# jcorsetti/oryon

Measured on AMD Instinct MI355X. Metric: image-pairs/sec end-to-end (feat+match+reg) @224², C=256; ADD(-S) parity, higher is better.
Workload: dtype f32

## Files before the change

include/oryon_hip.h:

```cpp
#ifndef ORYON_HIP_H
#define ORYON_HIP_H

#include <stddef.h>
#include <stdint.h>

#ifdef __cplusplus
extern "C" {
#endif

#define ORYON_OK 0
#define ORYON_ERR_INVALID_ARG (-1)
#define ORYON_ERR_HIP (-2)
#define ORYON_ERR_WORKSPACE (-3)
#define ORYON_ERR_NO_DEVICE (-4)
#define ORYON_ERR_STATE (-5)

#define ORYON_PAIR_OK 0
#define ORYON_PAIR_NO_MASK 1
#define ORYON_PAIR_NO_CORR 2

#define ORYON_MATCH_TILE 128

const char *oryon_version(void);
const char *oryon_last_error(void);
// ... 141 lines not shown
                     const float *cam_a, const float *cam_q, const int32_t *status, float *pcd_a, float *pcd_q,
                     int32_t *n_out, void *stream);

int oryon_lift_points(const float *depth, int H, int W, const float *cam9, const int32_t *x_idx, const int32_t *y_idx,
                      int n, float *out, void *stream);

int oryon_kabsch_batched(const float *A, const float *B, const float *w, int nb, int m, float *T, void *stream);

typedef struct oryon_pointdsc oryon_pointdsc_t;

typedef struct {
    int in_dim;
    int num_layers;
    int num_channels;
    int num_iterations;
    float ratio;
    float inlier_threshold;
    float sigma_d;
    int k;
    float nms_radius;
} oryon_pointdsc_config_t;

int oryon_pointdsc_create(oryon_pointdsc_t **handle, const oryon_pointdsc_config_t *cfg);
void oryon_pointdsc_destroy(oryon_pointdsc_t *handle);
int oryon_pointdsc_load_param(oryon_pointdsc_t *handle, const char *name, const float *data_host, int64_t numel);
int oryon_pointdsc_finalize(oryon_pointdsc_t *handle, void *stream);
size_t oryon_pointdsc_workspace_bytes(const oryon_pointdsc_t *handle, int B, int n_cap);
int oryon_pointdsc_register(oryon_pointdsc_t *handle, const float *src, const float *tgt, const int32_t *n, int B,
                            int n_cap, const int32_t *status_in, void *workspace, size_t workspace_bytes, float *T,
                            uint8_t *labels, int32_t *status_out, void *stream);
int oryon_pointdsc_encode(oryon_pointdsc_t *handle, const float *src, const float *tgt, const int32_t *n, int B,
                          int n_cap, void *workspace, size_t workspace_bytes, float *feat, float *confidence,
                          void *stream);
int oryon_pointdsc_seeds(oryon_pointdsc_t *handle, const float *src, const float *confidence, const int32_t *n, int B,
                         int n_cap, int S_cap, int32_t *seeds, int32_t *n_seeds, void *stream);
int oryon_pointdsc_hypotheses(oryon_pointdsc_t *handle, const float *src, const float *tgt, const float *feat,
                              const int32_t *n, const int32_t *seeds, const int32_t *n_seeds, int B, int n_cap,
                              int S_cap, void *workspace, size_t workspace_bytes, float *seed_T, float *fitness,
                              int32_t *best, void *stream);
int oryon_pointdsc_refine(oryon_pointdsc_t *handle, const float *src, const float *tgt, const int32_t *n, int B,
                          int n_cap, const float *T_in, float *T_out, uint8_t *labels, void *stream);

size_t oryon_ransac_workspace_bytes(int B, int n_cap, int max_iter);
int oryon_ransac_register(const float *src, const float *tgt, const int32_t *n, int B, int n_cap, int max_iter, double match_err,
                          double fix_percent, const int32_t *sample_idx, uint64_t seed, const int64_t *pair_key,
                          const int32_t *status_in, void *workspace, size_t workspace_bytes, float *T, int32_t *winner,
                          int32_t *exited, int32_t *counts, int32_t *status_out, void *stream);

size_t oryon_feature_loss_workspace_bytes(int B, int n_corr, int n_pool);
int oryon_feature_loss(const float *feat_a, const float *feat_q, int B, int C, int FH, int FW, const int32_t *corrs, int n_corr,
                       const int32_t *valid, const int32_t *pool, int n_pool, int pool_mode, float pos_margin, float neg_margin,
                       float neg_kernel, void *workspace, size_t workspace_bytes, float *d_pos, float *d_neg, int32_t *neg_idx,
                       float *pair_terms, float *losses, void *stream);
int oryon_mask_dice_sums(const float *logits, const int32_t *gt, int B, int H, int W, float threshold, double *sums, int32_t *mask,
                         int32_t *counts, void *stream);

size_t oryon_feature_loss_grad_workspace_bytes(int B, int C, int n_corr);
int oryon_feature_loss_grad(const float *feat_a, const float *feat_q, int B, int C, int FH, int FW, const int32_t *corrs, int n_corr,
                            const int32_t *valid, const int32_t *neg_idx, const float *d_pos, const float *d_neg, const float *g,
                            float pos_margin, float neg_margin, void *workspace, size_t workspace_bytes, float *grad_a, float *grad_q,
                            void *stream);
int oryon_mask_dice_grad(const float *logits, const int32_t *gt, int B, int H, int W, const double *sums, const float *g_mask,
                         float *grad_logits, void *stream);

typedef struct oryon_engine oryon_engine_t;
typedef struct {
    int B, C, FH, FW;
    int HA, WA, HQ, WQ;
    int layout;
    float dist_th;
    int n_corrs;
    int src_sampling;
    uint64_t seed;
    int round_f16;
    int n_slots;
    int overlap;
    int gather_sets;
    int reg_streams;
    int reg_lag;
    int screen;
    int sample_first;
    int x3_prefetch;
    int stream_roles;
    int solver;
    int ransac_max_iter;
    float ransac_match_err;
    float ransac_fix_percent;
} oryon_engine_config_t;
size_t oryon_engine_config_bytes(void);
size_t oryon_engine_arena_bytes(const oryon_engine_config_t *cfg, const oryon_pointdsc_t *solver);
int oryon_engine_create(oryon_engine_t **handle, const oryon_engine_config_t *cfg, oryon_pointdsc_t *solver, void *arena,
                        size_t arena_bytes);
void oryon_engine_destroy(oryon_engine_t *handle);
int oryon_engine_warm_streams(void);
int oryon_engine_set_stream_roles(oryon_engine_t *handle, int roles);
int oryon_engine_stream_roles(const oryon_engine_t *handle, int *roles);
int oryon_engine_buffer(const oryon_engine_t *handle, int slot, const char *name, size_t *offset, size_t *bytes);
int oryon_engine_geometry(const oryon_engine_t *handle, int *cap_a, int *cap_q, int *c_pad, int *n_cap);
int oryon_engine_submit(oryon_engine_t *handle, const float *feat_a, const float *feat_q, const int32_t *mask_a, const int32_t *mask_q,
                        const float *depth_a, const float *depth_q, const float *cam_a, const float *cam_q, const int64_t *pair_key,
                        int force_eager, int inputs_resident, void *caller_stream);
int oryon_engine_wait(oryon_engine_t *handle, int slot, void *caller_stream);
int oryon_engine_set_timing(oryon_engine_t *handle, int enable);
int oryon_engine_timing(oryon_engine_t *handle, int64_t step, float *out8);
int oryon_engine_elapsed(oryon_engine_t *handle, int64_t step_a, int event_a, int64_t step_b, int event_b, float *ms);
int oryon_engine_gather_ms(oryon_engine_t *handle, int64_t step, float *ms);
int oryon_engine_host_stats(const oryon_engine_t *handle, int64_t *n_submit, double *submit_ms_total, double *submit_ms_last);
int oryon_engine_x3_steps(const oryon_engine_t *handle, int64_t *n_steps);
int oryon_engine_feedback(oryon_engine_t *handle, int64_t *step, int64_t *n_undecided, int64_t *n_anchors);

int oryon_split_f16x3(const float *x, int64_t n, void *hi_f16, void *lo_f16, void *stream);
int oryon_x3_range_flag(int *value_out, int reset, void *stream);
int oryon_linear_f16x3(const float *A, int M, int K, const void *W_hi, const void *W_lo, const float *bias, int N, int act, float *C,
                       void *stream);
int oryon_linear_f16x3_acc(const float *A, int M, int K, const void *W_hi, const void *W_lo, const float *bias, int N, float *C,
                           void *stream);

int oryon_mha_f16x3(const float *qkv, int N, int L, int heads, int head_dim, float *out, void *stream);

int oryon_pose_metrics(const float *pred_pose, const float *gt_pose, int B, const float *model_pts, const int32_t *pts_offset, int n_models,
                       int max_pts, const int32_t *model_of_pair, float *workspace, float *out, void *stream);

size_t oryon_pose_bop_workspace_bytes(int B, int max_syms);
int oryon_pose_bop_errors(const double *pred_pose, const double *gt_pose, const double *K, int B, const double *model_pts_mm,
                          const int32_t *pts_offset, const double *syms, const int32_t *sym_offset, int n_models, int max_syms,
                          const int32_t *model_of_pair, int max_points, double *workspace, double *out, void *stream);

size_t oryon_render_depth_workspace_bytes(int N, int max_faces);
int oryon_render_depth(const float *pose, const float *K, int N, const float *verts_mm, const int32_t *vert_offset, const int32_t *faces,
                       const int32_t *face_offset, int n_models, int max_faces, const int32_t *model_of_image, int H, int W, void *workspace,
                       float *depth, void *stream);

size_t oryon_vsd_workspace_bytes(int B, int H, int W, int max_faces);
int oryon_vsd_counts(const double *pred_pose, const double *gt_pose, const double *K, const float *depth_test, int B, int H, int W,
                     const float *verts_mm, const int32_t *vert_offset, const int32_t *faces, const int32_t *face_offset, int n_models,
                     int max_faces, const int32_t *model_of_pair, const double *diameter_mm, double delta, const double *taus, int n_tau,
                     void *workspace, int32_t *counts, void *stream);

int oryon_gtc_lift(const float *depth, int B, int H, int W, const int32_t *pix, const int32_t *n, int cap, const double *cam9,
                   const double *pose, double *xyz, int32_t *yx, void *stream);
int oryon_pcd_nearest_f64(const double *src, const int32_t *n_src, const double *dst, const int32_t *n_dst, int B, int cap_src,
                          int cap_dst, int32_t *idx, double *d2, void *stream);
size_t oryon_gt_corrs_workspace_bytes(int B, int cap_a, int cap_q);
int oryon_gt_corrs(const float *depth_a, const float *depth_q, int B, int HA, int WA, int HQ, int WQ, const int32_t *pix_a,
                   const int32_t *n_a, int cap_a, const int32_t *pix_q, const int32_t *n_q, int cap_q, const double *cam_a,
                   const double *cam_q, const double *pose_aq, double threshold, const int32_t *status_in, void *workspace,
                   size_t workspace_bytes, int32_t *corrs, int32_t *n_corr, int32_t *idx, double *d2, void *stream);

typedef struct oryon_decoder oryon_decoder_t;
typedef struct {
    const float *gp_w[2], *gp_b[2];
    const float *up_w[3], *up_b[3];
    const float *c1_w[3];
    const float *n1_g[3], *n1_b[3];
    const float *c2_w[3];
    const float *n2_g[3], *n2_b[3];
    const float *head_w, *head_b;
} oryon_decoder_weights_t;
int oryon_decoder_create(const oryon_decoder_weights_t *weights, oryon_decoder_t **handle, void *stream);
void oryon_decoder_destroy(oryon_decoder_t *handle);
int64_t oryon_decoder_workspace_bytes(int n_img, int h, int w);
int oryon_decoder_workspace_layout(int n_img, int h, int w, int64_t *offsets3);
int oryon_decoder_forward(const oryon_decoder_t *handle, const float *x, const float *g2, const float *g3, int n_img, int h, int w,
                          void *workspace, int64_t workspace_bytes, float *featmap, float *logits, int guidance_layout, int stop_after, void *stream);

int oryon_fusion_window_attention_f32(const float *qk, const float *v, int B, int H, int W, int C, int heads, int window, int shift,
                                      float *out, void *stream);

int64_t oryon_conv24_image_bytes(int cout, int cin, int ksize);
int oryon_conv24_pack_f16x3(const float *w, int cout, int cin, int ksize, void *image, void *stream);
int oryon_conv24_f16x3(const float *x, int n, int cin, const void *image, const float *bias, int cout, int ksize, int relu, float *y, void *stream);

typedef struct {
    const float *ln1_w, *ln1_b, *wq, *bq, *wk, *bk, *wv, *bv, *ln2_w, *ln2_b, *w1, *b1, *w2, *b2;
} oryon_fusion_class_weights_t;
int oryon_fusion_class_layer_f32(const float *x, const float *text_guidance, const oryon_fusion_class_weights_t *weights, int B, float *out,
                                 void *stream);

#ifdef __cplusplus
}
#endif
#endif
```

oryon_amd/_lib.py:

```python
from __future__ import annotations

import ctypes
import os
from ctypes import POINTER, c_char_p, c_float, c_int, c_int64, c_size_t, c_uint64, c_void_p

import torch

_HERE = os.path.dirname(os.path.abspath(__file__))
LIB_PATH = os.path.join(_HERE, "liboryon_hip.so")
_lib = None


class OryonError(RuntimeError):
    pass


class EngineConfig(ctypes.Structure):
    _fields_ = [("B", c_int), ("C", c_int), ("FH", c_int), ("FW", c_int), ("HA", c_int), ("WA", c_int), ("HQ", c_int), ("WQ", c_int),
                ("layout", c_int), ("dist_th", c_float), ("n_corrs", c_int), ("src_sampling", c_int), ("seed", c_uint64),
                ("round_f16", c_int), ("n_slots", c_int), ("overlap", c_int), ("gather_sets", c_int), ("reg_streams", c_int), ("reg_lag", c_int), ("screen", c_int), ("sample_first", c_int), ("x3_prefetch", c_int), ("stream_roles", c_int),
                ("solver", c_int), ("ransac_max_iter", c_int), ("ransac_match_err", c_float), ("ransac_fix_percent", c_float)]


class DecoderWeights(ctypes.Structure):
    _fields_ = [("gp_w", c_void_p * 2), ("gp_b", c_void_p * 2), ("up_w", c_void_p * 3), ("up_b", c_void_p * 3), ("c1_w", c_void_p * 3),
                ("n1_g", c_void_p * 3), ("n1_b", c_void_p * 3), ("c2_w", c_void_p * 3), ("n2_g", c_void_p * 3), ("n2_b", c_void_p * 3),
                ("head_w", c_void_p), ("head_b", c_void_p)]


class FusionClassWeights(ctypes.Structure):
    _fields_ = [(n, c_void_p) for n in ("ln1_w", "ln1_b", "wq", "bq", "wk", "bk", "wv", "bv", "ln2_w", "ln2_b", "w1", "b1", "w2", "b2")]


class PointDSCConfig(ctypes.Structure):
    _fields_ = [("in_dim", c_int), ("num_layers", c_int), ("num_channels", c_int), ("num_iterations", c_int),
                ("ratio", c_float), ("inlier_threshold", c_float), ("sigma_d", c_float), ("k", c_int),
                ("nms_radius", c_float)]


_P = c_void_p
_PROTOS = {
    "oryon_version": (c_char_p, []),
    "oryon_last_error": (c_char_p, []),
    "oryon_device_check": (c_int, [c_int]),
    "oryon_profile_events": (c_int, [_P, _P]),
    "oryon_dominant_kernel": (c_char_p, []),
    "oryon_quick_gelu_bf16": (c_int, [_P, _P, ctypes.c_int64, _P]),
    "oryon_add_layernorm_bf16": (c_int, [_P, _P, _P, _P, ctypes.c_int64, c_int, c_float, _P, _P, _P]),
    "oryon_add_layernorm_f32": (c_int, [_P, _P, _P, _P, ctypes.c_int64, c_int, c_float, _P, _P, _P]),
    "oryon_swin_window_attention_bf16": (c_int, [_P, _P, _P, c_int, c_int, c_int, c_int, c_int, c_int, _P, _P]),
    "oryon_swin_window_attention_f32": (c_int, [_P, _P, _P, c_int, c_int, c_int, c_int, c_int, c_int, _P, _P]),
    "oryon_round_to_f16_f32": (c_int, [_P, _P, ctypes.c_int64, _P]),
    "oryon_rgb_resize_bilinear": (c_int, [_P, c_int, c_int, c_int, c_int, c_int, _P, _P]),
    "oryon_resize_bilinear_f32": (c_int, [_P, c_int, c_int, c_int, c_int, c_int, c_int, _P, _P]),
    "oryon_rgb_augment_workspace_bytes": (c_size_t, [c_int]),
    "oryon_rgb_augment_resize": (c_int, [_P, _P, c_int, c_int, c_int, c_int, c_int, _P, c_size_t, _P, _P]),
    "oryon_resize_bilinear_f32_flip": (c_int, [_P, _P, c_int, c_int, c_int, c_int, c_int, c_int, _P, _P]),
    "oryon_mask_resize_nearest_flip": (c_int, [_P, _P, c_int, c_int, c_int, c_int, c_int, _P, _P]),
    "oryon_roi_compact": (c_int, [_P, c_int, c_int, _P, _P, _P]),
    "oryon_mask_from_logits": (c_int, [_P, c_int64, c_float, _P, _P]),
    "oryon_mask_resize_nearest": (c_int, [_P, c_int, c_int, c_int, c_int, c_int, _P, _P]),
    "oryon_roi_subsample": (c_int, [_P, _P, c_int, c_int, c_int, c_uint64, _P, _P]),
    "oryon_gather_normalise_f32": (c_int, [_P, c_int, c_int, c_int, _P, c_int, _P, c_int, c_int, _P, _P, _P]),
    "oryon_match_workspace_bytes": (c_size_t, [c_int, c_int]),
    "oryon_match_f32": (c_int, [_P, _P, c_int, c_int, c_int, c_int, _P, _P, c_float, _P, _P, _P, _P, c_size_t, _P]),
    "oryon_match_screened_workspace_bytes": (c_size_t, [c_int, c_int, c_int]),
    "oryon_gather_normalise_q8": (c_int, [_P, c_int, c_int, c_int, _P, c_int, _P, c_int, c_int, _P, _P, _P, _P, _P, _P]),
    "oryon_gather_q8": (c_int, [_P, c_int, c_int, c_int, c_int, _P, c_int, _P, c_int, c_int, _P, _P, _P, _P, _P, c_int, _P]),
    "oryon_match_screened8_raw_workspace_bytes": (c_size_t, [c_int, c_int, c_int, c_int]),
    "oryon_match_screened8_raw": (c_int, [_P, _P, _P, _P, c_int, c_int, c_int, _P, c_int, _P, _P, _P, _P, c_int, c_int, c_int, c_int,
                                          _P, _P, c_float, _P, _P, _P, _P, c_int, _P, c_size_t, _P]),
    "oryon_match_corrs_i8_workspace_bytes": (c_size_t, [c_int, c_int, c_int, c_int, c_int]),
    "oryon_match_corrs_i8": (c_int, [_P, _P, _P, _P, c_int, c_int, c_int, _P, c_int, _P, c_int, _P, _P, _P, _P, c_int, c_int, c_int, c_int,
                                     _P, _P, c_float, c_int, c_int, c_int, c_uint64, _P, c_int, _P, _P, _P, _P, _P, _P, _P, _P, c_int, _P,
                                     c_size_t, _P]),
    "oryon_x3_range_flag": (c_int, [POINTER(c_int), c_int, _P]),
    "oryon_gather_mx6": (c_int, [_P, c_int, c_int, c_int, c_int, _P, c_int, _P, c_int, c_int, _P, _P, _P, _P, c_int, _P]),
    "oryon_match_corrs_mx6": (c_int, [_P, _P, _P, _P, c_int, c_int, c_int, _P, c_int, _P, c_int, _P, _P, _P, c_int, c_int, c_int, c_int,
                                      _P, _P, c_float, c_int, c_int, c_int, c_uint64, _P, _P, _P, _P, _P, _P, _P, _P, _P, c_int, _P,
                                      c_size_t, _P]),
    "oryon_gather_mx6_x3": (c_int, [_P, c_int, c_int, c_int, c_int, _P, c_int, _P, c_int, c_int, _P, _P, _P, _P, _P, c_int, _P]),
    "oryon_match_corrs_mx6_x3": (c_int, [_P, _P, _P, _P, c_int, c_int, c_int, _P, c_int, _P, c_int, _P, _P, _P, _P, _P, c_int, c_int, c_int, c_int,
                                         _P, _P, c_float, c_int, c_int, c_int, c_uint64, _P, _P, _P, _P, _P, _P, _P, _P, _P, c_int, _P,
                                         c_size_t, _P]),
    "oryon_match_corrs_i8_araw": (c_int, [_P, _P, _P, _P, _P, c_int, c_int, c_int, _P, c_int, _P, c_int, _P, _P, _P, _P, c_int, c_int, c_int,
                                          c_int, _P, _P, c_float, c_int, c_int, c_int, c_uint64, _P, _P, _P, _P, _P, _P, _P, _P, _P, c_int,
                                          _P, c_size_t, _P]),
    "oryon_match_corrs_mx6_araw": (c_int, [_P, _P, _P, _P, _P, c_int, c_int, c_int, _P, c_int, _P, c_int, _P, _P, _P, c_int, c_int, c_int,
                                           c_int, _P, _P, c_float, c_int, c_int, c_int, c_uint64, _P, _P, _P, _P, _P, _P, _P, _P, _P, c_int,
                                           _P, c_size_t, _P]),
    "oryon_match_corrs_mx6_x3_araw": (c_int, [_P, _P, _P, _P, _P, c_int, c_int, c_int, _P, c_int, _P, c_int, _P, _P, _P, _P, _P, c_int, c_int,
                                              c_int, c_int, _P, _P, c_float, c_int, c_int, c_int, c_uint64, _P, _P, _P, _P, _P, _P, _P, _P,
                                              _P, c_int, _P, c_size_t, _P]),
    "oryon_match_screened8_workspace_bytes": (c_size_t, [c_int, c_int, c_int, c_int]),
    "oryon_match_screened8": (c_int, [_P, _P, _P, _P, _P, _P, _P, c_int, c_int, c_int, c_int, c_int, _P, _P, c_float, _P, _P, _P,
                                      _P, _P, c_size_t, _P]),
    "oryon_match_screened": (c_int, [_P, _P, _P, _P, c_int, c_int, c_int, c_int, _P, _P, c_float, _P, _P, _P, _P, c_size_t, _P]),
    "oryon_sample_first_gate": (c_int, [_P, _P, _P, c_int, c_int, _P, _P]),
    "oryon_sample_first_merge": (c_int, [_P, _P, _P, _P, _P, c_int, c_int, _P, _P, _P, _P, _P]),
    "oryon_select_corrs": (c_int, [_P, _P, c_int, c_int, _P, _P, _P, _P, c_int, c_int, c_int, c_int, c_int, c_uint64, _P, _P,
                                   _P, _P, _P, _P, _P]),
    "oryon_lift_pairs": (c_int, [_P, _P, c_int, c_int, c_int, c_int, _P, c_int, c_int, _P, c_int, c_int, _P, _P, _P, _P,
                                 _P, _P, _P]),
    "oryon_lift_points": (c_int, [_P, c_int, c_int, _P, _P, _P, c_int, _P, _P]),
    "oryon_kabsch_batched": (c_int, [_P, _P, _P, c_int, c_int, _P, _P]),
    "oryon_split_f16x3": (c_int, [_P, c_int64, _P, _P, _P]),
    "oryon_linear_f16x3": (c_int, [_P, c_int, c_int, _P, _P, _P, c_int, c_int, _P, _P]),
    "oryon_linear_f16x3_acc": (c_int, [_P, c_int, c_int, _P, _P, _P, c_int, _P, _P]),
    "oryon_mha_f16x3": (c_int, [_P, c_int, c_int, c_int, c_int, _P, _P]),
    "oryon_pose_metrics": (c_int, [_P, _P, c_int, _P, _P, c_int, c_int, _P, _P, _P, _P]),
    "oryon_pose_bop_workspace_bytes": (c_size_t, [c_int, c_int]),
    "oryon_pose_bop_errors": (c_int, [_P, _P, _P, c_int, _P, _P, _P, _P, c_int, c_int, _P, c_int, _P, _P, _P]),
    "oryon_render_depth_workspace_bytes": (c_size_t, [c_int, c_int]),
    "oryon_render_depth": (c_int, [_P, _P, c_int, _P, _P, _P, _P, c_int, c_int, _P, c_int, c_int, _P, _P, _P]),
    "oryon_vsd_workspace_bytes": (c_size_t, [c_int, c_int, c_int, c_int]),
    "oryon_vsd_counts": (c_int, [_P, _P, _P, _P, c_int, c_int, c_int, _P, _P, _P, _P, c_int, c_int, _P, _P, ctypes.c_double, _P, c_int,
                                 _P, _P, _P]),
    "oryon_engine_arena_bytes": (c_size_t, [POINTER(EngineConfig), c_void_p]),
    "oryon_engine_create": (c_int, [POINTER(c_void_p), POINTER(EngineConfig), c_void_p, _P, c_size_t]),
    "oryon_engine_destroy": (None, [c_void_p]),
    "oryon_engine_warm_streams": (c_int, []),
    "oryon_engine_set_stream_roles": (c_int, [c_void_p, c_int]),
    "oryon_engine_stream_roles": (c_int, [c_void_p, POINTER(c_int)]),
    "oryon_engine_buffer": (c_int, [c_void_p, c_int, c_char_p, POINTER(c_size_t), POINTER(c_size_t)]),
    "oryon_engine_geometry": (c_int, [c_void_p, POINTER(c_int), POINTER(c_int), POINTER(c_int), POINTER(c_int)]),
    "oryon_engine_submit": (c_int, [c_void_p, _P, _P, _P, _P, _P, _P, _P, _P, _P, c_int, c_int, _P]),
    "oryon_engine_wait": (c_int, [c_void_p, c_int, _P]),
    "oryon_engine_set_timing": (c_int, [c_void_p, c_int]),
    "oryon_engine_timing": (c_int, [c_void_p, c_int64, POINTER(c_float)]),
    "oryon_engine_elapsed": (c_int, [c_void_p, c_int64, c_int, c_int64, c_int, POINTER(c_float)]),
    "oryon_engine_gather_ms": (c_int, [c_void_p, c_int64, POINTER(c_float)]),
    "oryon_engine_config_bytes": (c_size_t, []),
    "oryon_engine_host_stats": (c_int, [c_void_p, POINTER(c_int64), POINTER(ctypes.c_double), POINTER(ctypes.c_double)]),
    "oryon_engine_x3_steps": (c_int, [c_void_p, POINTER(c_int64)]),
    "oryon_engine_feedback": (c_int, [_P, POINTER(c_int64), POINTER(c_int64), POINTER(c_int64)]),
    "oryon_fusion_window_attention_f32": (c_int, [_P, _P, c_int, c_int, c_int, c_int, c_int, c_int, c_int, _P, _P]),
    "oryon_fusion_class_layer_f32": (c_int, [_P, _P, POINTER(FusionClassWeights), c_int, _P, _P]),
    "oryon_conv24_image_bytes": (c_int64, [c_int, c_int, c_int]),
    "oryon_conv24_pack_f16x3": (c_int, [_P, c_int, c_int, c_int, _P, _P]),
    "oryon_conv24_f16x3": (c_int, [_P, c_int, c_int, _P, _P, c_int, c_int, c_int, _P, _P]),
    "oryon_decoder_create": (c_int, [POINTER(DecoderWeights), POINTER(c_void_p), _P]),
    "oryon_decoder_destroy": (None, [c_void_p]),
    "oryon_decoder_workspace_bytes": (c_int64, [c_int, c_int, c_int]),
    "oryon_decoder_workspace_layout": (c_int, [c_int, c_int, c_int, POINTER(c_int64)]),
    "oryon_decoder_forward": (c_int, [c_void_p, _P, _P, _P, c_int, c_int, c_int, _P, c_int64, _P, _P, c_int, c_int, _P]),
    "oryon_pointdsc_create": (c_int, [POINTER(c_void_p), POINTER(PointDSCConfig)]),
    "oryon_pointdsc_destroy": (None, [c_void_p]),
    "oryon_pointdsc_load_param": (c_int, [c_void_p, c_char_p, _P, c_int64]),
    "oryon_pointdsc_finalize": (c_int, [c_void_p, _P]),
    "oryon_pointdsc_workspace_bytes": (c_size_t, [c_void_p, c_int, c_int]),
    "oryon_pointdsc_register": (c_int, [c_void_p, _P, _P, _P, c_int, c_int, _P, _P, c_size_t, _P, _P, _P, _P]),
    "oryon_ransac_workspace_bytes": (c_size_t, [c_int, c_int, c_int]),
    "oryon_ransac_register": (c_int, [_P, _P, _P, c_int, c_int, c_int, ctypes.c_double, ctypes.c_double, _P, c_uint64, _P, _P, _P, c_size_t,
                                      _P, _P, _P, _P, _P, _P]),
    "oryon_feature_loss_workspace_bytes": (c_size_t, [c_int, c_int, c_int]),
    "oryon_feature_loss": (c_int, [_P, _P, c_int, c_int, c_int, c_int, _P, c_int, _P, _P, c_int, c_int, c_float, c_float, c_float, _P, c_size_t,
                                   _P, _P, _P, _P, _P, _P]),
    "oryon_mask_dice_sums": (c_int, [_P, _P, c_int, c_int, c_int, c_float, _P, _P, _P, _P]),
    "oryon_feature_loss_grad_workspace_bytes": (c_size_t, [c_int, c_int, c_int]),
    "oryon_feature_loss_grad": (c_int, [_P, _P, c_int, c_int, c_int, c_int, _P, c_int, _P, _P, _P, _P, _P, c_float, c_float, _P, c_size_t,
                                        _P, _P, _P]),
    "oryon_mask_dice_grad": (c_int, [_P, _P, c_int, c_int, c_int, _P, _P, _P, _P]),
    "oryon_pointdsc_encode": (c_int, [c_void_p, _P, _P, _P, c_int, c_int, _P, c_size_t, _P, _P, _P]),
    "oryon_pointdsc_seeds": (c_int, [c_void_p, _P, _P, _P, c_int, c_int, c_int, _P, _P, _P]),
    "oryon_pointdsc_hypotheses": (c_int, [c_void_p, _P, _P, _P, _P, _P, _P, c_int, c_int, c_int, _P, c_size_t, _P, _P,
                                          _P, _P]),
    "oryon_pointdsc_refine": (c_int, [c_void_p, _P, _P, _P, c_int, c_int, _P, _P, _P, _P]),
    "oryon_gtc_lift": (c_int, [_P, c_int, c_int, c_int, _P, _P, c_int, _P, _P, _P, _P, _P]),
    "oryon_pcd_nearest_f64": (c_int, [_P, _P, _P, _P, c_int, c_int, c_int, _P, _P, _P]),
    "oryon_gt_corrs_workspace_bytes": (c_size_t, [c_int, c_int, c_int]),
    "oryon_gt_corrs": (c_int, [_P, _P, c_int, c_int, c_int, c_int, c_int, _P, _P, c_int, _P, _P, c_int, _P, _P, _P, ctypes.c_double, _P,
                               _P, c_size_t, _P, _P, _P, _P, _P]),
}

EXPORTS = tuple(_PROTOS)


def lib():
    global _lib
    if _lib is None:
        if not os.path.exists(LIB_PATH):
            raise OryonError(f"{LIB_PATH} not found: build it with `python -c 'import __graft_entry__ as g; g.build()'` "
                             "or `make -C oryon_amd/csrc` - there is no CPU fallback")
        L = ctypes.CDLL(LIB_PATH)
        missing = [name for name in _PROTOS if not hasattr(L, name)]
        if missing:
            raise OryonError(f"{LIB_PATH} lacks symbols declared in include/oryon_hip.h: {missing} (stale build?)")
        for name, (res, args) in _PROTOS.items():
            fn = getattr(L, name)
            fn.restype = res
            fn.argtypes = args
        if L.oryon_engine_config_bytes() != ctypes.sizeof(EngineConfig):
            raise OryonError(f"{LIB_PATH}: oryon_engine_config_t is {L.oryon_engine_config_bytes()} bytes in the library, "
                             f"{ctypes.sizeof(EngineConfig)} in oryon_amd/_lib.py (stale build?)")
        _lib = L
    return _lib


def check(code: int, what: str = "") -> None:
    if code != 0:
        raise OryonError(f"{what or 'liboryon_hip'} failed ({code}): {lib().oryon_last_error().decode()}")


def ptr(t) -> int | None:
    if t is None:
        return None
    assert t.is_contiguous(), "C ABI takes contiguous buffers"
    return t.data_ptr()


def stream_ptr(device=None) -> int:
    return torch.cuda.current_stream(device).cuda_stream


def require_gpu(device) -> torch.device:
    dev = torch.device(device)
    if dev.type != "cuda" or not torch.cuda.is_available():
# ... 5 lines not shown
```

oryon_amd/csrc/engine.hip:

```cpp
#include <stdlib.h>
#include <chrono>
#include <new>
#include <vector>
#include "common.h"
#include "match_common.h"

using namespace oryon;

namespace {
constexpr int MAX_SLOTS = 8;
constexpr int MAX_G_SLOTS = 4;
constexpr int MAX_REG_STREAMS = 4;
constexpr int TIMING_RING = 64;
constexpr int ROW_PAD = 256;
constexpr int POOL_STREAMS = 8;
constexpr int DEFAULT_ROLES = 2345;

inline bool roles_valid(int roles)
{
    if (roles < 0 || roles > 7777) return false;
    for (int d = 0, r = roles; d < 4; ++d, r /= 10)
        if (r % 10 >= POOL_STREAMS) return false;
    return true;
}

inline size_t up(size_t x, size_t m) { return (x + m - 1) / m * m; }

struct GatherBuf {
    int8_t *a8, *q8;
    float *a_sc, *q_sc, *a_eps, *q_eps, *a_norm, *q_norm, *a_hat;
    void *q_hilo;
    float *q_lo_max;
    int8_t *a8_1;
    float *a_sc_1, *a_eps_1, *a_norm_1;
};

struct SlotBuf {
    int32_t *roi_a, *roi_q, *n_a, *n_q;
    float *min_dist;
    int32_t *argmin;
    uint8_t *valid;
    int32_t *corrs, *n_valid, *n_sel, *status, *n_und;
    int32_t *roi_a1, *n_a1, *n_a2, *corrs2, *n_valid2, *n_sel2, *status2;
    float *pcd_a, *pcd_q;
    int32_t *n_lift;
    float *pose;
    int32_t *status_out;
    int32_t *n_valid_out, *n_lift_out;
    void *pdsc_ws;
    size_t base, bytes;
};

struct Named {
    const char *name;
    size_t off, bytes;
};

struct Layout {
    GatherBuf gbuf[MAX_G_SLOTS];
    SlotBuf slot[MAX_SLOTS];
    std::vector<Named> names[MAX_SLOTS];
    void *match_ws;
    size_t match_ws_bytes, pdsc_ws_bytes, bytes;
    int cap_a, cap_q, c_pad, n_cap, cap_a1;
};
}

struct oryon_engine {
    oryon_engine_config_t cfg;
    oryon_pointdsc_t *solver;
    char *arena;
    Layout L;
    int device;
    hipStream_t sg, sm, sr[MAX_REG_STREAMS];
    int n_reg_streams;
    int roles;
    hipEvent_t ev_inputs[MAX_SLOTS], ev_gathered[MAX_SLOTS], ev_matched[MAX_SLOTS], ev_done[MAX_SLOTS];
    hipEvent_t tev[TIMING_RING][9];
    bool timed[TIMING_RING];
    bool used[MAX_SLOTS];
    bool timing;
    int32_t *fb_host;
    hipEvent_t ev_fb[MAX_SLOTS];
    int64_t fb_step[MAX_SLOTS];
    int64_t fb_seen;
    bool hard_mode;
// ... 35 lines not shown
        TAKE(a_sc, float, B * (L.cap_a / 16));
        TAKE(q_sc, float, B * (L.cap_q / 16));
        TAKE(a_eps, float, B);
        TAKE(q_eps, float, B);
        TAKE(a_norm, float, B * L.cap_a);
        TAKE(q_norm, float, B * L.cap_q);
        TAKE(a_hat, float, B * L.cap_a * L.c_pad);
        b.q_hilo = nullptr;
        b.q_lo_max = nullptr;
        if (c.x3_prefetch && L.c_pad == 256) {
            b.q_hilo = take((size_t)2 * B * L.cap_q * L.c_pad * 2);
            TAKE(q_lo_max, float, B);
        }
        b.a8_1 = nullptr;
        b.a_sc_1 = b.a_eps_1 = b.a_norm_1 = nullptr;
        if (L.cap_a1) {
            TAKE(a8_1, int8_t, B * L.cap_a1 * L.c_pad);
            TAKE(a_sc_1, float, B * (L.cap_a1 / 16));
            TAKE(a_eps_1, float, B);
            TAKE(a_norm_1, float, B * L.cap_a1);
        }
#undef TAKE
    }
    for (int s = 0; s < c.n_slots; ++s) {
        SlotBuf &b = L.slot[s];
        L.names[s].clear();
        b.base = off;
        auto take = [&](const char *name, size_t n) {
            const size_t o = off;
            off = up(off + n, 256);
            L.names[s].push_back({name, o, n});
            return base ? base + o : nullptr;
        };
#define TAKE(field, type, count) b.field = reinterpret_cast<type *>(take(#field, (size_t)(count) * sizeof(type)))
        TAKE(roi_a, int32_t, B * HW);
        TAKE(roi_q, int32_t, B * HW);
        TAKE(n_a, int32_t, B);
        TAKE(n_q, int32_t, B);
        TAKE(min_dist, float, B * L.cap_a);
        TAKE(argmin, int32_t, B * L.cap_a);
        TAKE(valid, uint8_t, B * L.cap_a);
        TAKE(corrs, int32_t, B * L.n_cap * 4);
        TAKE(n_valid, int32_t, B);
        TAKE(n_sel, int32_t, B);
        TAKE(status, int32_t, B);
        TAKE(n_und, int32_t, B);
        b.roi_a1 = b.n_a1 = b.n_a2 = b.corrs2 = b.n_valid2 = b.n_sel2 = b.status2 = nullptr;
        if (L.cap_a1) {
            TAKE(roi_a1, int32_t, B * HW);
            TAKE(n_a1, int32_t, B);
            TAKE(n_a2, int32_t, B);
            TAKE(corrs2, int32_t, B * L.n_cap * 4);
            TAKE(n_valid2, int32_t, B);
            TAKE(n_sel2, int32_t, B);
            TAKE(status2, int32_t, B);
        }
        TAKE(pcd_a, float, B * L.n_cap * 3);
        TAKE(pcd_q, float, B * L.n_cap * 3);
        TAKE(n_lift, int32_t, B);
        TAKE(pose, float, B * 16);
        TAKE(status_out, int32_t, B);
        TAKE(n_valid_out, int32_t, B);
        TAKE(n_lift_out, int32_t, B);
#undef TAKE
        b.pdsc_ws = take("pdsc_ws", L.pdsc_ws_bytes);
        b.bytes = off - b.base;
    }
    L.match_ws = base ? base + off : nullptr;
    off = up(off + L.match_ws_bytes, 256);
    L.bytes = off;
    return ORYON_OK;
}

int check_cfg(const oryon_engine_config_t *c)
{
    ORYON_CHECK_ARG(c && c->B > 0 && c->C > 0 && c->C <= 512 && c->FH > 0 && c->FW > 0);
    ORYON_CHECK_ARG(c->HA > 0 && c->WA > 0 && c->HQ > 0 && c->WQ > 0 && c->n_corrs > 0 && c->src_sampling >= 0);
    ORYON_CHECK_ARG(c->dist_th > 0.0f && c->dist_th <= 0.5f && c->n_slots >= 1 && c->n_slots <= MAX_SLOTS);
    ORYON_CHECK_ARG(c->gather_sets >= 1 && c->gather_sets <= MAX_G_SLOTS && c->gather_sets <= c->n_slots);
    ORYON_CHECK_ARG(c->reg_streams >= 1 && c->reg_streams <= MAX_REG_STREAMS && c->reg_lag >= 0 && c->reg_lag < c->n_slots);
    ORYON_CHECK_ARG((c->layout == ORYON_LAYOUT_NCHW || c->layout == ORYON_LAYOUT_NHWC) && (c->screen == 0 || c->screen == 1));
    ORYON_CHECK_ARG(c->overlap >= 0 && c->overlap <= 2 && (c->overlap == 0 || c->n_slots >= 2));
    ORYON_CHECK_ARG((size_t)c->C * (size_t)c->FH * (size_t)c->FW * 4u < (1ull << 32));
    ORYON_CHECK_ARG(c->sample_first >= 0 && (c->x3_prefetch == 0 || c->x3_prefetch == 1));
    ORYON_CHECK_ARG(roles_valid(c->stream_roles));
    ORYON_CHECK_ARG(c->solver == 0 || (c->solver == 1 && c->ransac_max_iter > 0 && c->ransac_match_err >= 0.0f));
    return ORYON_OK;
}
}

namespace oryon {
__global__ void engine_counts_kernel(const int32_t *__restrict__ n_valid, const int32_t *__restrict__ n_lift, int B,
                                     int32_t *__restrict__ n_valid_out, int32_t *__restrict__ n_lift_out)
{
    const int i = blockIdx.x * blockDim.x + threadIdx.x;
    if (i < B) {
        n_valid_out[i] = n_valid[i];
        n_lift_out[i] = n_lift[i];
    }
}
}

extern "C" size_t oryon_engine_config_bytes(void) { return sizeof(oryon_engine_config_t); }

extern "C" size_t oryon_engine_arena_bytes(const oryon_engine_config_t *cfg, const oryon_pointdsc_t *solver)
{
    if (check_cfg(cfg) || (!solver && cfg->solver != 1)) return 0;
    Layout L;
    if (carve_engine(*cfg, solver, nullptr, L)) return 0;
    return L.bytes;
}

namespace oryon {
__global__ void pool_touch_kernel() {}
struct StreamPool { hipStream_t all[POOL_STREAMS] = {nullptr, nullptr, nullptr, nullptr, nullptr, nullptr, nullptr, nullptr}; };
static std::mutex g_pool_mu;
static StreamPool g_pools[64];
static hipError_t acquire_pool(int dev, hipStream_t out[POOL_STREAMS])
{
    std::lock_guard<std::mutex> lock(g_pool_mu);
    StreamPool &pool = g_pools[(dev >= 0 && dev < 64) ? dev : 0];
    for (int i = 0; i < POOL_STREAMS; ++i) {
        if (!pool.all[i]) {
            hipError_t err = hipStreamCreateWithFlags(&pool.all[i], hipStreamNonBlocking);
            if (err != hipSuccess) { pool.all[i] = nullptr; return err; }
            hipLaunchKernelGGL(pool_touch_kernel, dim3(1), dim3(64), 0, pool.all[i]);
            err = hipStreamSynchronize(pool.all[i]);
            if (err != hipSuccess) return err;
        }
        out[i] = pool.all[i];
    }
    return hipSuccess;
}
}

extern "C" int oryon_engine_warm_streams(void)
{
    int dev = 0;
    ORYON_CHECK_HIP(hipGetDevice(&dev));
    hipStream_t tmp[POOL_STREAMS];
    ORYON_CHECK_HIP(acquire_pool(dev, tmp));
    return ORYON_OK;
}

namespace {
int assign_roles(oryon_engine *e, int roles)
{
    hipStream_t pool[POOL_STREAMS];
    ORYON_CHECK_HIP(acquire_pool(e->device, pool));
    const int r_m = roles / 1000 % 10, r_g = roles / 100 % 10, r_r0 = roles / 10 % 10, r_r1 = roles % 10;
    e->sm = e->cfg.overlap >= 1 ? pool[r_m] : nullptr;
    e->sg = e->cfg.overlap >= 2 ? pool[r_g] : nullptr;
    for (int s = 0; s < MAX_REG_STREAMS; ++s) e->sr[s] = nullptr;
    for (int s = 0; s < e->n_reg_streams; ++s)
        if (e->cfg.overlap >= 1) e->sr[s] = pool[(s == 0 ? r_r0 : s == 1 ? r_r1 : 2 + s) & 7];
    e->roles = roles;
    return ORYON_OK;
}
}

extern "C" int oryon_engine_create(oryon_engine_t **handle, const oryon_engine_config_t *cfg, oryon_pointdsc_t *solver, void *arena,
                                   size_t arena_bytes)
{
    ORYON_CHECK_ARG(handle && arena);
    int rc = check_cfg(cfg);
    if (rc) return rc;
    ORYON_CHECK_ARG(solver || cfg->solver == 1);
// ... 193 lines not shown
                long und = 0, all = 0;
                for (int i = 0; i < B; ++i) { und += h[i]; all += h[B + i]; }
                e->hard_mode = all > 0 && 4 * und > all;
                e->fb_seen = e->fb_step[s];
            }
        }
        x3_pre = e->hard_mode && !sf && g.q_hilo != nullptr;
    }
    if (x3_pre) a_hat_k0 = g.a_hat;
    if (timing) ORYON_CHECK_HIP(hipEventRecord(tev[8], sg));
    if (ablate & 1) {
    } else if (mx6) {
        if (x3_pre) {
            if ((rc = oryon_gather_mx6_x3(feat_q, B, c.C, HW, c.layout, b.roi_q, HW, b.n_q, e->L.cap_q, e->L.c_pad, reinterpret_cast<uint8_t *>(g.q8),
                                          g.q_eps, g.q_norm, g.q_hilo, g.q_lo_max, c.round_f16, sg))) return rc;
            e->n_x3 += 1;
        } else
        if ((rc = oryon_gather_mx6(feat_q, B, c.C, HW, c.layout, b.roi_q, HW, b.n_q, e->L.cap_q, e->L.c_pad, reinterpret_cast<uint8_t *>(g.q8),
                                   g.q_eps, g.q_norm, nullptr, c.round_f16, sg))) return rc;
        if ((rc = oryon_gather_mx6(feat_a, B, c.C, HW, c.layout, roi_a_k0, HW, n_a_k0, cap_a_k0, e->L.c_pad, reinterpret_cast<uint8_t *>(a8_k0),
                                   a_eps_k0, a_norm_k0, a_hat_k0, c.round_f16, sg))) return rc;
    } else {
    if ((rc = oryon_gather_q8(feat_q, B, c.C, HW, c.layout, b.roi_q, HW, b.n_q, e->L.cap_q, e->L.c_pad, g.q8, g.q_sc, g.q_eps, g.q_norm,
                              nullptr, c.round_f16, sg))) return rc;
    if ((rc = oryon_gather_q8(feat_a, B, c.C, HW, c.layout, roi_a_k0, HW, n_a_k0, cap_a_k0, e->L.c_pad, a8_k0, a_sc_k0, a_eps_k0, a_norm_k0,
                              a_hat_k0, c.round_f16, sg))) return rc;
    }
    if (timing) ORYON_CHECK_HIP(hipEventRecord(tev[1], sg));
    if (sg != sm) {
        ORYON_CHECK_HIP(hipEventRecord(e->ev_gathered[slot], sg));
        ORYON_CHECK_HIP(hipStreamWaitEvent(sm, e->ev_gathered[slot], 0));
    }
    struct Disarm {
        bool armed = false;
        ~Disarm() { if (armed) (void)oryon_profile_events(nullptr, nullptr); }
    } disarm;
    if (timing) {
        ORYON_CHECK_HIP(hipEventRecord(tev[2], sm));
        (void)oryon_profile_events(tev[4], tev[5]);
        disarm.armed = true;
    }
    auto match_call = [&](const float *a_norm_, const int8_t *a8_, const float *a_sc_, const float *a_eps_, const int32_t *roi_a_, int cap_a_,
                          const int32_t *n_a_, int32_t *corrs_, int32_t *n_valid_, int32_t *n_sel_, int32_t *status_, int32_t *n_und_) -> int {
        MatchCorrsArgs m;
        m.a_i8 = a8_;
        m.a_scale = mx6 ? a_eps_ : a_sc_;
        m.roi_a = roi_a_;
        m.roi_stride_a = HW;
        m.feat_q = feat_q;
        m.q_norm = g.q_norm;
        m.roi_q = b.roi_q;
        m.roi_stride_q = HW;
        m.q_i8 = g.q8;
        m.q_scale = mx6 ? nullptr : g.q_sc;
        m.q_eps_max = g.q_eps;
        m.C_true = c.C;
        m.HW = HW;
        m.layout = c.layout;
        m.B = B;
        m.C = e->L.c_pad;
        m.cap_a = cap_a_;
        m.cap_q = e->L.cap_q;
        m.round_f16 = c.round_f16;
        m.n_a = n_a_;
        m.n_q = b.n_q;
        m.threshold = c.dist_th;
        m.W = c.FW;
        m.max_corrs = c.n_corrs;
        m.corr_rows = e->L.n_cap;
        m.seed = c.seed;
        m.pair_key = pair_key;
        m.min_dist = b.min_dist;
        m.argmin = b.argmin;
        m.valid = b.valid;
        m.corrs = corrs_;
        m.n_valid = n_valid_;
        m.n_sel = n_sel_;
        m.status = status_;
        m.n_undecided = n_und_;
        m.workspace = e->L.match_ws;
        m.workspace_bytes = e->L.match_ws_bytes;
        m.stream = sm;
        m.fmt = mx6 ? 1 : 0;
        if (mx6 && x3_pre) {
            m.a_hat = g.a_hat;
            m.q_hi_lo = g.q_hilo;
            m.q_lo_sq_max = g.q_lo_max;
        } else if (force_eager) {
            m.a_hat = g.a_hat;
            m.force_eager = force_eager;
        } else {
            m.feat_a = feat_a;
            m.a_norm = a_norm_;
        }
        return match_corrs_lazy_impl(m);
    };
    if (ablate & 2) {
    } else if (sf) {
        if ((rc = match_call(g.a_norm_1, g.a8_1, g.a_sc_1, g.a_eps_1, b.roi_a1, e->L.cap_a1, b.n_a1, b.corrs, b.n_valid, b.n_sel, b.status, b.n_und)))
            return rc;
        if ((rc = oryon_sample_first_gate(b.n_valid, b.n_a1, b.n_a, B, c.n_corrs, b.n_a2, sm))) return rc;
        if (mx6) {
            if ((rc = oryon_gather_mx6(feat_a, B, c.C, HW, c.layout, b.roi_a, HW, b.n_a2, e->L.cap_a, e->L.c_pad, reinterpret_cast<uint8_t *>(g.a8),
                                       g.a_eps, g.a_norm, nullptr, c.round_f16, sm))) return rc;
        } else if ((rc = oryon_gather_q8(feat_a, B, c.C, HW, c.layout, b.roi_a, HW, b.n_a2, e->L.cap_a, e->L.c_pad, g.a8, g.a_sc, g.a_eps, g.a_norm,
                                         nullptr, c.round_f16, sm))) return rc;
        if ((rc = match_call(g.a_norm, g.a8, g.a_sc, g.a_eps, b.roi_a, e->L.cap_a, b.n_a2, b.corrs2, b.n_valid2, b.n_sel2, b.status2, nullptr)))
            return rc;
        if ((rc = oryon_sample_first_merge(b.n_a2, b.corrs2, b.n_valid2, b.n_sel2, b.status2, B, e->L.n_cap, b.corrs, b.n_valid, b.n_sel, b.status,
                                           sm))) return rc;
    } else if ((rc = match_call(g.a_norm, g.a8, g.a_sc, g.a_eps, b.roi_a, e->L.cap_a, b.n_a, b.corrs, b.n_valid, b.n_sel, b.status, b.n_und)))
        return rc;
    if (e->fb_host && mx6 && !(ablate & 2)) {
        int32_t *h = e->fb_host + (size_t)slot * 2 * B;
        ORYON_CHECK_HIP(hipMemcpyAsync(h, b.n_und, (size_t)B * sizeof(int32_t), hipMemcpyDeviceToHost, sm));
        ORYON_CHECK_HIP(hipMemcpyAsync(h + B, b.n_a, (size_t)B * sizeof(int32_t), hipMemcpyDeviceToHost, sm));
        ORYON_CHECK_HIP(hipEventRecord(e->ev_fb[slot], sm));
        e->fb_step[slot] = e->n_submit;
    }
    if (!(ablate & 2) && (rc = oryon_lift_pairs(b.corrs, b.n_sel, B, e->L.n_cap, c.FH, c.FW, depth_a, c.HA, c.WA, depth_q, c.HQ, c.WQ, cam_a, cam_q,
                                                b.status, b.pcd_a, b.pcd_q, b.n_lift, sm))) return rc;
    if (timing) ORYON_CHECK_HIP(hipEventRecord(tev[3], sm));
    if (c.overlap >= 1) {
        ORYON_CHECK_HIP(hipEventRecord(e->ev_matched[slot], sm));
        ORYON_CHECK_HIP(hipStreamWaitEvent(sr, e->ev_matched[slot], 0));
    }
    if (timing) ORYON_CHECK_HIP(hipEventRecord(tev[6], sr));
    if (c.solver == 1) {
        if (!(ablate & 4) && (rc = oryon_ransac_register(b.pcd_a, b.pcd_q, b.n_lift, B, e->L.n_cap, c.ransac_max_iter, (double)c.ransac_match_err,
                                                         (double)c.ransac_fix_percent, nullptr, c.seed, pair_key, b.status, b.pdsc_ws,
                                                         e->L.pdsc_ws_bytes, b.pose, nullptr, nullptr, nullptr, b.status_out, sr))) return rc;
    } else if (!(ablate & 4) && (rc = oryon_pointdsc_register(e->solver, b.pcd_a, b.pcd_q, b.n_lift, B, e->L.n_cap, b.status, b.pdsc_ws, e->L.pdsc_ws_bytes,
                                                       b.pose, nullptr, b.status_out, sr))) return rc;
    hipLaunchKernelGGL(engine_counts_kernel, dim3((B + 255) / 256), dim3(256), 0, sr, b.n_valid, b.n_lift, B, b.n_valid_out, b.n_lift_out);
    ORYON_CHECK_LAUNCH();
    if (timing) ORYON_CHECK_HIP(hipEventRecord(tev[7], sr));
    if (c.overlap >= 1) ORYON_CHECK_HIP(hipEventRecord(e->ev_done[slot], sr));
    e->used[slot] = true;
    e->n_submit += 1;
    e->host_ns_last = std::chrono::duration<double, std::nano>(std::chrono::steady_clock::now() - t_host0).count();
    e->host_ns_total += e->host_ns_last;
    return slot;
}

extern "C" int oryon_engine_wait(oryon_engine_t *e, int slot, void *caller_stream)
{
    ORYON_CHECK_ARG(e && slot >= 0 && slot < e->cfg.n_slots && e->used[slot]);
    if (e->cfg.overlap >= 1) ORYON_CHECK_HIP(hipStreamWaitEvent(as_stream(caller_stream), e->ev_done[slot], 0));
    return ORYON_OK;
}

extern "C" int oryon_engine_host_stats(const oryon_engine_t *e, int64_t *n_submit, double *submit_ms_total, double *submit_ms_last)
{
    ORYON_CHECK_ARG(e);
    if (n_submit) *n_submit = e->n_submit;
    if (submit_ms_total) *submit_ms_total = e->host_ns_total * 1e-6;
    if (submit_ms_last) *submit_ms_last = e->host_ns_last * 1e-6;
    return ORYON_OK;
}

extern "C" int oryon_engine_feedback(oryon_engine_t *e, int64_t *step, int64_t *n_undecided, int64_t *n_anchors)
{
    ORYON_CHECK_ARG(e && step && n_undecided && n_anchors);
    *step = -1;
    *n_undecided = *n_anchors = 0;
    if (!e->fb_host) return ORYON_OK;
    const int B = e->cfg.B;
    int best = -1;
    for (int s = 0; s < e->cfg.n_slots; ++s)
        if (e->fb_step[s] >= 0 && (best < 0 || e->fb_step[s] > e->fb_step[best]) && hipEventQuery(e->ev_fb[s]) == hipSuccess) best = s;
    if (best < 0) return ORYON_OK;
    const int32_t *h = e->fb_host + (size_t)best * 2 * B;
    int64_t und = 0, all = 0;
    for (int i = 0; i < B; ++i) { und += h[i]; all += h[B + i]; }
    *step = e->fb_step[best];
    *n_undecided = und;
    *n_anchors = all;
    return ORYON_OK;
}

extern "C" int oryon_engine_x3_steps(const oryon_engine_t *e, int64_t *n_steps)
{
    ORYON_CHECK_ARG(e && n_steps);
    *n_steps = e->n_x3;
    return ORYON_OK;
}

extern "C" int oryon_engine_timing(oryon_engine_t *e, int64_t step, float *out8)
{
    ORYON_CHECK_ARG(e && out8 && step >= 0 && step < e->n_submit && step >= e->n_submit - TIMING_RING);
    if (!e->timed[step % TIMING_RING]) { set_error("oryon_engine_timing: step %lld was submitted with timing off (oryon_engine_set_timing)", (long long)step); return ORYON_ERR_STATE; }
    hipEvent_t *t = e->tev[step % TIMING_RING];
    const int q[8][2] = {{0, 1}, {2, 3}, {4, 5}, {6, 7}, {0, 2}, {0, 3}, {0, 6}, {0, 7}};
    for (int i = 0; i < 8; ++i) {
        const hipError_t err = hipEventElapsedTime(&out8[i], t[q[i][0]], t[q[i][1]]);
        if (err != hipSuccess) {
            set_error("oryon_engine_timing: %s (step still running?)", hipGetErrorString(err));
            return ORYON_ERR_STATE;
        }
    }
    return ORYON_OK;
}

extern "C" int oryon_engine_gather_ms(oryon_engine_t *e, int64_t step, float *ms)
{
    ORYON_CHECK_ARG(e && ms && step >= 0 && step < e->n_submit && step >= e->n_submit - TIMING_RING);
    if (!e->timed[step % TIMING_RING]) { set_error("oryon_engine_gather_ms: step %lld was submitted with timing off", (long long)step); return ORYON_ERR_STATE; }
    const hipError_t err = hipEventElapsedTime(ms, e->tev[step % TIMING_RING][8], e->tev[step % TIMING_RING][1]);
    if (err != hipSuccess) { set_error("oryon_engine_gather_ms: %s (step still running?)", hipGetErrorString(err)); return ORYON_ERR_STATE; }
    return ORYON_OK;
}

extern "C" int oryon_engine_elapsed(oryon_engine_t *e, int64_t step_a, int event_a, int64_t step_b, int event_b, float *ms)
{
    ORYON_CHECK_ARG(e && ms && event_a >= 0 && event_a < 8 && event_b >= 0 && event_b < 8);
    for (int64_t st : {step_a, step_b}) {
        ORYON_CHECK_ARG(st >= 0 && st < e->n_submit && st >= e->n_submit - TIMING_RING);
        if (!e->timed[st % TIMING_RING]) { set_error("oryon_engine_elapsed: step %lld was submitted with timing off", (long long)st); return ORYON_ERR_STATE; }
    }
    const hipError_t err = hipEventElapsedTime(ms, e->tev[step_a % TIMING_RING][event_a], e->tev[step_b % TIMING_RING][event_b]);
    if (err != hipSuccess) { set_error("oryon_engine_elapsed: %s (step still running?)", hipGetErrorString(err)); return ORYON_ERR_STATE; }
    return ORYON_OK;
}
```

oryon_amd/csrc/match_common.h:

```cpp
#pragma once
#include <hip/hip_fp16.h>
#include <type_traits>
#include "common.h"

namespace oryon {

typedef float f32x16 __attribute__((ext_vector_type(16)));

__device__ __forceinline__ void lex_min(float &d, int &i, float od, int oi)
{
    const bool take = (od < d) || (od == d && oi < i);
    d = take ? od : d;
    i = take ? oi : i;
}

int match_f32_flagged(const float *a_hat, const float *q_hat, int B, int C, int cap_a, int cap_q, const int32_t *n_a,
                      const int32_t *n_q, float threshold, float *min_dist, int32_t *argmin, uint8_t *valid,
                      const int32_t *panel_flag, const uint8_t *row_flag, void *stream);

size_t match_x3_scratch_bytes(int B, int cap_s, int S, int cap_q);
int match_x3_resolve(const float *a_c, const int32_t *n_c, int cap_s, const float *feat_q, int C_true, int HW, int layout,
                     const int32_t *roi_q, int roi_stride_q, const float *q_norm, const int32_t *n_q, int B, int cap_q, float threshold,
                     int round_f16, __half *qh, __half *ql, __half *ah, __half *al, void *scratch, float *md_c, int32_t *am_c, uint8_t *va_c,
                     int32_t **n_ovf_out, int32_t **ovf_idx_out, const int32_t *orig_idx, int orig_stride, const int32_t *sid_final, int cap_a,
                     const __half *q_hi_lo_pre, const float *q_lo_sq_max_pre, hipStream_t st);
void match_x3_scatter_ovf(int B, int cap_s, const int32_t *n_ovf, const int32_t *ovf_idx, const float *md_o, const int32_t *am_o,
                          const uint8_t *va_o, float *md_c, int32_t *am_c, uint8_t *va_c, hipStream_t st);

const char *screen_mx6_name(int C);
void launch_screen_mx6(int C, int groups, int T, hipStream_t st, const uint8_t *a6, const uint8_t *q6, int B, int cap_a, int cap_q,
                       const int32_t *n_a, const int32_t *n_q, int S, float *ws_max, int32_t *ws_i1, float *ws_m2, int C_true,
                       int cascade = 0, const int32_t *gate = nullptr, int win = 0);
inline int mx6_panels_per_pair(int cap_a) { return (cap_a + 1023) / 1024; }
void launch_screen_mx6_sampled(hipStream_t st, const uint8_t *a6_panel, const uint8_t *q6, int B, int cap_q, const int32_t *n_rows,
                               const int32_t *n_q, int S, float *ws_max, int32_t *ws_i1, float *ws_m2, int C_true);
constexpr int MX6_SAMPLED_PANEL = 512;
inline int mx6_sampled_splits(int B) { int s = (512 + B - 1) / B; return s < 1 ? 1 : s > 16 ? 16 : s; }

struct Carver {
    char *base;
    size_t off;
    explicit Carver(void *b, size_t start = 0) : base(static_cast<char *>(b)), off(start) {}
    template <class T> void operator()(T *&p, size_t count)
    {
        p = base ? reinterpret_cast<T *>(base + off) : nullptr;
        off = (off + count * sizeof(std::conditional_t<std::is_void<T>::value, char, T>) + 255) / 256 * 256;
    }
};

constexpr int MT16 = 256;

struct ScreenWs {
    float *ws_max, *ws_m2, *m_final, *amb_max;
    int32_t *ws_i1, *cnt, *cand, *panel_flag, *n_amb, *amb_idx;
    __half *a16c;
    uint8_t *row_flag;
    size_t zero_off, zero_bytes;
};
struct Screen8Ws : ScreenWs {
    __half *q16;
    float *a_hat_c, *md_c;
    int32_t *am_c;
    uint8_t *va_c;
    void *nested;
    size_t nested_bytes;
};
struct Screen8RawWs : Screen8Ws {
    float *q_hat, *scale_scratch, *eps_scratch;
    int8_t *q8_scratch;
    int32_t *need_f32;
};
int pick_split16(int B, int T);
size_t carve_screen8_raw(void *base, Screen8RawWs &w, int B, int C, int cap_a, int cap_q, int S);

int gather_q8_launch(const float *feat, int n_maps, int C, int HW, int layout, const int32_t *roi, int roi_stride, const int32_t *count,
                     const int32_t *map_enable, int rows_cap, int C_pad, int8_t *out8, float *scale, float *eps, float *norm,
                     float *out32, int lanes_per_row, int round_f16, hipStream_t st, int fmt = 0, void *aux = nullptr);
int select_corrs_launch(const int32_t *roi_a, const int32_t *roi_q, int roi_stride_a, int roi_stride_q, const int32_t *n_a,
                        const int32_t *n_q, const int32_t *argmin, const uint8_t *valid, int cap_a, int B, int W, int max_corrs,
                        int corr_rows, uint64_t seed, const int64_t *pair_key, int32_t *scratch, int32_t *corrs, int32_t *n_valid,
                        int32_t *n_sel, int32_t *status, int32_t *sel_rows, const int32_t *pair_eager, hipStream_t st);

struct Screen8Args {
    const float *a_hat = nullptr;
    const int8_t *a_i8 = nullptr;
    const int8_t *q_i8 = nullptr;
    const float *a_scale = nullptr;
    const float *q_scale = nullptr;
    const float *q_eps_max = nullptr;
    int B = 0;
    int C_true = 0;
    int C = 0;
    int cap_a = 0;
    int cap_q = 0;
    const int32_t *n_q = nullptr;
    float threshold = 0.0f;
    const float *feat_q = nullptr;
    int HW = 0;
    int layout = 0;
    const int32_t *roi_q = nullptr;
    int roi_stride_q = 0;
    const float *q_norm = nullptr;
    int round_f16 = 0;
    float *min_dist = nullptr;
    int32_t *argmin = nullptr;
    uint8_t *valid = nullptr;
    void *stream = nullptr;
};
inline int check_launch(const char *who)
{
    const hipError_t e = hipGetLastError();
    if (e == hipSuccess) return ORYON_OK;
    set_error("%s: launch failed: %s", who, hipGetErrorString(e));
    return ORYON_ERR_HIP;
}
void screen8_step(const Screen8Args &m, int S, const int32_t *n_a, const ScreenWs &w);
void decide8_step(const Screen8Args &m, int S, const int32_t *n_a, const ScreenWs &w);
void rescore_raw_step(const Screen8Args &m, const int32_t *n_a, int rescore_lanes, const Screen8RawWs &w);
int screen16_fallback(const Screen8Args &m, const float *q_hat, const Screen8Ws &w, const char *who);
int raw_fallbacks(const Screen8Args &m, const int32_t *n_a, const Screen8RawWs &w, const char *who, const char *entry);

struct MatchCorrsArgs : Screen8Args {
    const float *feat_a = nullptr;
    const float *a_norm = nullptr;
    const int32_t *roi_a = nullptr;
    int roi_stride_a = 0;
    const void *q_hi_lo = nullptr;
    const float *q_lo_sq_max = nullptr;
    const int32_t *n_a = nullptr;
    int W = 0;
    int max_corrs = 0;
    int corr_rows = 0;
    uint64_t seed = 0;
    const int64_t *pair_key = nullptr;
    int32_t *corrs = nullptr;
    int32_t *n_valid = nullptr;
    int32_t *n_sel = nullptr;
    int32_t *status = nullptr;
    int32_t *n_undecided = nullptr;
    void *workspace = nullptr;
    size_t workspace_bytes = 0;
    int fmt = 0;
    int force_eager = 0;
};
int match_corrs_lazy_impl(const MatchCorrsArgs &m);

}
```

oryon_amd/csrc/match_corrs.hip:

```cpp
#include <hip/hip_fp16.h>
#include "common.h"
#include "match_common.h"

namespace oryon {
constexpr uint8_t LZ_INVALID = 0, LZ_VALID = 1, LZ_UNCERTAIN = 2, LZ_AMB_VALID = 3, LZ_RESOLVED = 4, LZ_AMB_UNCERTAIN = 5;

__global__ __launch_bounds__(256) void match_decide_lite_kernel(
    int cap_a, const int32_t *__restrict__ n_a, int S, const float *__restrict__ ws_m1, const int32_t *__restrict__ ws_i1,
    const float *__restrict__ ws_m2, const float *__restrict__ a_scale8, const float *__restrict__ eps_q8, float cut0, float sqrt_c,
    float c_true, int force_eager, int fmt, int x3, float *__restrict__ m_final, int32_t *__restrict__ sid_final, float *__restrict__ margin_out,
    uint8_t *__restrict__ state, uint8_t *__restrict__ valid, float *__restrict__ min_dist, int32_t *__restrict__ argmin,
    int32_t *__restrict__ pair_eager, int32_t *__restrict__ n_unc, int32_t *__restrict__ unc_idx, int32_t *__restrict__ n_ambu,
    int32_t *__restrict__ ambu_idx, int32_t *__restrict__ need_f32_lazy, int32_t *__restrict__ n_amb_total)
{
    const int p = blockIdx.y, a = blockIdx.x * 256 + threadIdx.x;
    if (a >= n_a[p]) return;
    const size_t arow = (size_t)p * cap_a + a;
    float m1 = -INFINITY, m2 = -INFINITY;
    int sid = 0;
    for (int s = 0; s < S; ++s) {
        const size_t o = ((size_t)p * S + s) * cap_a + a;
        const float x1 = ws_m1[o], x2 = ws_m2[o];
        m2 = fmaxf(fminf(m1, x1), fmaxf(m2, x2));
        if (x1 > m1) { m1 = x1; sid = ws_i1[o]; }
// ... 85 lines not shown
                                                                   uint8_t *__restrict__ state)
{
    const int p = blockIdx.y, sl = blockIdx.x * 256 + threadIdx.x;
    const int n = count[p] < cap_c ? count[p] : cap_c;
    if (sl >= n) return;
    const size_t src = (size_t)p * cap_c + sl, dst = (size_t)p * cap_a + idx[(size_t)p * idx_stride + sl];
    min_dist[dst] = md_c[src];
    argmin[dst] = am_c[src];
    valid[dst] = va_c[src];
    state[dst] = LZ_RESOLVED;
}

__global__ __launch_bounds__(256) void match_list_sampled_amb_kernel(int cap_a, const uint8_t *__restrict__ state,
                                                                      const int32_t *__restrict__ pair_eager, const int32_t *__restrict__ n_sel,
                                                                      const int32_t *__restrict__ sel_rows, int corr_rows,
                                                                      int32_t *__restrict__ mark, int32_t *__restrict__ n_list,
                                                                      int32_t *__restrict__ list)
{
    __shared__ int wave_cnt[4];
    const int p = blockIdx.x;
    if (pair_eager[p]) return;
    const int n = n_sel[p], t = threadIdx.x, lane = t & 63, wave = t >> 6;
    for (int s = t; s < n; s += 256) {
        const int a = sel_rows[(size_t)p * corr_rows + s];
        if (state[(size_t)p * cap_a + a] == LZ_AMB_VALID) mark[(size_t)p * cap_a + a] = 1;
    }
    __threadfence_block();
    __syncthreads();
    const int R = (cap_a + 255) / 256;
    const int32_t *mk = mark + (size_t)p * cap_a;
    int mine = 0;
    for (int i = 0; i < R; ++i) {
        const int a = t * R + i;
        mine += (a < cap_a && mk[a] != 0) ? 1 : 0;
    }
    int incl = mine;
#pragma unroll
    for (int off = 1; off < 64; off <<= 1) {
        const int v = __shfl_up(incl, off);
        if (lane >= off) incl += v;
    }
    if (lane == 63) wave_cnt[wave] = incl;
    __syncthreads();
    int off0 = incl - mine;
    for (int w = 0; w < wave; ++w) off0 += wave_cnt[w];
    for (int i = 0; i < R; ++i) {
        const int a = t * R + i;
        if (a < cap_a && mk[a] != 0) list[(size_t)p * corr_rows + off0++] = a;
    }
    if (t == 255) n_list[p] = off0;
}

__global__ __launch_bounds__(256) void match_panel_settle_kernel(int cap_a, int T8, int S, const int32_t *__restrict__ n_a,
                                                                  const float *__restrict__ ws_m1, float *__restrict__ ws_m2,
                                                                  const float *__restrict__ a_err, const float *__restrict__ q_err,
                                                                  float cut0, int32_t *__restrict__ gate)
{
    __shared__ int bad;
    const int p = blockIdx.y, panel = blockIdx.x, t = threadIdx.x;
    const int na = n_a[p], a0 = panel * 1024;
    if (a0 >= na) return;
    if (t == 0) bad = 0;
    __syncthreads();
    const float ea = a_err[p], eq = q_err[p];
    const float delta = ea + eq + ea * eq + 1.2e-4f;
    const float thr = delta < 0.2f ? cut0 + delta + 2e-5f : INFINITY;
    int mine = 0;
    for (int a = a0 + t; a < a0 + 1024 && a < na; a += 256) {
        float m1 = -INFINITY;
        for (int s_ = 0; s_ < S; ++s_) m1 = fmaxf(m1, ws_m1[((size_t)p * S + s_) * cap_a + a]);
        mine |= !(m1 > thr);
    }
    if (mine) atomicOr(&bad, 1);
    __syncthreads();
    const int open = bad;
    if (t == 0) gate[p * T8 + panel] = open;
    if (!open)
        for (int a = a0 + t; a < a0 + 1024 && a < na; a += 256)
            for (int s_ = 0; s_ < S; ++s_) ws_m2[((size_t)p * S + s_) * cap_a + a] = INFINITY;
}

__global__ __launch_bounds__(256) void match_compact_rows_kernel(const uint8_t *__restrict__ rows, int row_bytes, int cap_a, int cap_c,
                                                                  const int32_t *__restrict__ count, const int32_t *__restrict__ idx,
                                                                  int idx_stride, uint8_t *__restrict__ out)
{
    const int p = blockIdx.y, sl = blockIdx.x * 16 + (threadIdx.x >> 4), l = threadIdx.x & 15;
    if (sl >= cap_c) return;
    const int n = count[p] < cap_c ? count[p] : cap_c;
    uint4 *d = reinterpret_cast<uint4 *>(out + ((size_t)p * cap_c + sl) * row_bytes);
    if (sl >= n) {
        for (int i = l; i < row_bytes / 16; i += 16) d[i] = make_uint4(0, 0, 0, 0);
        return;
    }
    const uint4 *src = reinterpret_cast<const uint4 *>(rows + ((size_t)p * cap_a + idx[(size_t)p * idx_stride + sl]) * row_bytes);
    for (int i = l; i < row_bytes / 16; i += 16) d[i] = src[i];
}

__global__ __launch_bounds__(256) void match_decide_sampled_kernel(int cap_a, int cap_c, int S, const int32_t *__restrict__ count,
                                                                    const int32_t *__restrict__ idx, int idx_stride,
                                                                    const float *__restrict__ ws_m1, const int32_t *__restrict__ ws_i1,
                                                                    const float *__restrict__ ws_m2, const float *__restrict__ a_err,
                                                                    const float *__restrict__ q_err, float *__restrict__ m_final,
                                                                    int32_t *__restrict__ sid_final, float *__restrict__ margin_out,
                                                                    uint8_t *__restrict__ state, int32_t *__restrict__ mark,
                                                                    int32_t *__restrict__ count_before)
{
    const int p = blockIdx.y, sl = blockIdx.x * 256 + threadIdx.x;
    const int n = count[p] < cap_c ? count[p] : cap_c;
    if (sl == 0) count_before[p] = n;
    if (sl >= n) return;
    const int a = idx[(size_t)p * idx_stride + sl];
    float m1 = -INFINITY, m2 = -INFINITY;
    int sid = 0;
    for (int s = 0; s < S; ++s) {
        const size_t o = ((size_t)p * S + s) * cap_c + sl;
        const float x1 = ws_m1[o], x2 = ws_m2[o];
        m2 = fmaxf(fminf(m1, x1), fmaxf(m2, x2));
        if (x1 > m1) { m1 = x1; sid = ws_i1[o]; }
    }
    const float ea = a_err[p], eq = q_err[p];
    const float delta = ea + eq + ea * eq + 1.2e-4f;
    const float margin = delta < 0.2f ? 2.0f * delta + 2e-7f : INFINITY;
    const size_t arow = (size_t)p * cap_a + a;
    m_final[arow] = m1;
    sid_final[arow] = sid;
    margin_out[arow] = margin;
    if (m1 - m2 > margin) {
        state[arow] = LZ_VALID;
        mark[arow] = 0;
    }
}

typedef float f32x32r __attribute__((ext_vector_type(32)));
typedef unsigned u32x6r __attribute__((ext_vector_type(6)));

__device__ __forceinline__ float mx6_block_dot(const uint4 a_lo, const uint4 a_up, const uint4 q_lo, const uint4 q_up)
{
    const u32x6r ca = {a_lo.x, a_lo.y, a_lo.z, a_lo.w, a_up.x, a_up.y}, cq = {q_lo.x, q_lo.y, q_lo.z, q_lo.w, q_up.x, q_up.y};
    const f32x32r fa = __builtin_amdgcn_cvt_scalef32_pk32_f32_fp6(ca, 1.0f), fq = __builtin_amdgcn_cvt_scalef32_pk32_f32_fp6(cq, 1.0f);
    float sum = 0.0f;
#pragma unroll
    for (int i = 0; i < 32; ++i) sum = __fmaf_rn(fa[i], fq[i], sum);
    return sum * ldexpf(1.0f, (int)(a_up.z & 255u) + (int)(q_up.z & 255u) - 254);
}

struct AnchorRaw {
    const float *feat_a;
    const int32_t *roi_a;
    const float *a_norm;
    int roi_stride;
};

template <bool NHWC>
__device__ __forceinline__ float anchor_raw_unit(const float *__restrict__ fa, int pix, float d, int k, int C_true, int HW, int round_f16)
{
    float x = 0.0f;
    if (k < C_true) x = NHWC ? fa[(size_t)pix * C_true + k] : fa[(size_t)k * HW + pix];
    if (round_f16) x = __half2float(__float2half_rn(x));
    return __fdiv_rn(x, d);
}

template <bool NHWC, bool NEED_DIST = true, int FMT = 0>
__device__ __forceinline__ void resolve_anchor(int p, int a, const float *__restrict__ a_hat, const AnchorRaw &araw, const int8_t *__restrict__ a8,
                                               const int8_t *__restrict__ q8, const float *__restrict__ q_scale8,
                                               const float *__restrict__ a_scale8, const float *__restrict__ feat_q, int C_true, int HW,
                                               const int32_t *__restrict__ roi_q, int roi_stride, const float *__restrict__ norm_q,
                                               int Cp, int cap_a, int cap_q, int nq, float m1, int sid, float margin, float *lds ,
                                               int round_f16, float &d_out, int &j_out)
{
    const int lane = threadIdx.x & 63;
    const size_t arow = (size_t)p * cap_a + a;
    const int half = sid & 1, blk = sid >> 1;
    const int r = lane >> 2, seg = lane & 3;
    const int q = blk * 32 + (r & 3) + 8 * (r >> 2) + 4 * half;
    bool hit;
    if constexpr (FMT == 1) {
        float s6 = 0.0f;
        if (q < nq) {
            const uint4 *ar = reinterpret_cast<const uint4 *>(a8 + arow * Cp) + seg * (Cp / 64);
            const uint4 *qr = reinterpret_cast<const uint4 *>(q8 + ((size_t)p * cap_q + q) * Cp) + seg * (Cp / 64);
            for (int b = 0; b < Cp / 128; ++b) s6 += mx6_block_dot(ar[2 * b], ar[2 * b + 1], qr[2 * b], qr[2 * b + 1]);
        }
        s6 += __shfl_xor(s6, 1);
        s6 += __shfl_xor(s6, 2);
        float mx = (q < nq) ? s6 : -INFINITY;
        mx = fmaxf(mx, __shfl_xor(mx, 4));
        mx = fmaxf(mx, __shfl_xor(mx, 8));
        mx = fmaxf(mx, __shfl_xor(mx, 16));
        mx = fmaxf(mx, __shfl_xor(mx, 32));
        hit = (seg == 0) && (q < nq) && (s6 >= mx - margin - 4e-5f);
        (void)m1;
    } else {
    const float sa = a_scale8[(size_t)p * (cap_a / 16) + (a >> 5) * 2 + ((a >> 2) & 1)];
    int idot = 0;
    if (q < nq) {
        const uint4 *ar = reinterpret_cast<const uint4 *>(a8 + arow * Cp) + seg * (Cp / 64);
        const uint4 *qr = reinterpret_cast<const uint4 *>(q8 + ((size_t)p * cap_q + q) * Cp) + seg * (Cp / 64);
        for (int i0 = 0; i0 < Cp / 64; ++i0) {
            const uint4 av = ar[i0], qv = qr[i0];
            idot = __builtin_amdgcn_sdot4((int)av.x, (int)qv.x, idot, false);
            idot = __builtin_amdgcn_sdot4((int)av.y, (int)qv.y, idot, false);
            idot = __builtin_amdgcn_sdot4((int)av.z, (int)qv.z, idot, false);
            idot = __builtin_amdgcn_sdot4((int)av.w, (int)qv.w, idot, false);
        }
    }
    idot += __shfl_xor(idot, 1);
    idot += __shfl_xor(idot, 2);
    const float s8 = (float)idot * q_scale8[(size_t)p * (cap_q / 16) + sid] * sa;
    hit = (seg == 0) && (q < nq) && (s8 >= m1 - margin);
    }
    unsigned long long hits = __ballot(hit);
    if (!NEED_DIST && __popcll(hits) == 1) {
        j_out = __shfl(q, __ffsll((long long)hits) - 1);
// ... 87 lines not shown
    const float *__restrict__ m_final, const int32_t *__restrict__ sid_final, const float *__restrict__ margin_in,
    const int32_t *__restrict__ n_unc, const int32_t *__restrict__ unc_idx, const int32_t *__restrict__ pair_eager,
    uint8_t *__restrict__ state, uint8_t *__restrict__ valid, float *__restrict__ min_dist, int32_t *__restrict__ argmin, int round_f16)
{
    extern __shared__ float lds_res[];
    const int p = blockIdx.y;
    if (pair_eager[p]) return;
    const int wave = threadIdx.x >> 6, lane = threadIdx.x & 63;
    const int n = n_unc[p];
    for (int i = blockIdx.x * 4 + wave; i < n; i += gridDim.x * 4) {
        const int a = unc_idx[(size_t)p * cap_a + i];
        const size_t arow = (size_t)p * cap_a + a;
        float d;
        int j;
        resolve_anchor<NHWC, true, FMT>(p, a, a_hat, araw, a8, q8, q_scale8, a_scale8, feat_q, C_true, HW, roi_q, roi_stride, norm_q, Cp, cap_a, cap_q, n_q[p],
                             m_final[arow], sid_final[arow], margin_in[arow], lds_res + wave * 2 * Cp, round_f16, d, j);
        if (lane == 0) {
            min_dist[arow] = d;
            argmin[arow] = j;
            valid[arow] = (d < thr) ? 1 : 0;
            state[arow] = LZ_RESOLVED;
        }
    }
}

template <bool NHWC, int FMT = 0>
__global__ __launch_bounds__(256) void match_resolve_selected_kernel(
    const float *__restrict__ a_hat, const AnchorRaw araw, const int8_t *__restrict__ a8, const int8_t *__restrict__ q8, const float *__restrict__ q_scale8,
    const float *__restrict__ a_scale8, const float *__restrict__ feat_q, int C_true, int HW, const int32_t *__restrict__ roi_q,
    int roi_stride, const float *__restrict__ norm_q, int Cp, int cap_a, int cap_q, const int32_t *__restrict__ n_q, int W,
    const float *__restrict__ m_final, const int32_t *__restrict__ sid_final, const float *__restrict__ margin_in,
    const uint8_t *__restrict__ state, const int32_t *__restrict__ pair_eager, const int32_t *__restrict__ n_sel,
    const int32_t *__restrict__ sel_rows, int corr_rows, float *__restrict__ min_dist, int32_t *__restrict__ argmin,
    int32_t *__restrict__ corrs, int round_f16)
{
    extern __shared__ float lds_res[];
    const int p = blockIdx.y;
    if (pair_eager[p]) return;
    const int wave = threadIdx.x >> 6, lane = threadIdx.x & 63;
    const int slot = blockIdx.x * 4 + wave;
    if (slot >= n_sel[p]) return;
    const int a = sel_rows[(size_t)p * corr_rows + slot];
    const size_t arow = (size_t)p * cap_a + a;
    float d = 0.0f;
    int j;
    if (state[arow] == LZ_RESOLVED) {
        j = argmin[arow];
    } else {
        resolve_anchor<NHWC, false, FMT>(p, a, a_hat, araw, a8, q8, q_scale8, a_scale8, feat_q, C_true, HW, roi_q, roi_stride, norm_q, Cp, cap_a, cap_q,
                                    n_q[p], m_final[arow], sid_final[arow], margin_in[arow], lds_res + wave * 2 * Cp, round_f16, d, j);
        if (lane == 0) {
            argmin[arow] = j;
            if (d == d) min_dist[arow] = d;
        }
    }
    if (lane == 0) {
        j = (j < 0 || j >= n_q[p]) ? 0 : j;
        const int pq = roi_q[(size_t)p * roi_stride + j];
        corrs[((size_t)p * corr_rows + slot) * 4 + 2] = pq / W;
        corrs[((size_t)p * corr_rows + slot) * 4 + 3] = pq % W;
    }
}
}

using namespace oryon;

namespace {
struct LazyWs : Screen8RawWs {
    float *margin;
    int32_t *sid_final, *pair_eager, *n_unc, *unc_idx, *n_a_eager, *n_a_lazy, *sel_rows, *scratch;
    int32_t *n_ambu, *ambu_idx, *n_ambv, *ambv_idx, *need_f32_lazy, *n_amb_total, *mark;
    void *exact_ws;
    size_t exact_ws_bytes;
    __half *x3_ah, *x3_al;
    float *x3_a_ovf, *x3_md_o;
    int32_t *x3_am_o;
    uint8_t *x3_va_o;
    void *x3_scratch;
    uint8_t *state;
    uint8_t *cs_panel;
    float *cs_max, *cs_m2;
    int32_t *cs_i1;
    int32_t *n_ambv0, *cs_gate;
    size_t lazy_zero_off, lazy_zero_bytes;
};

int sampled_cap(int corr_rows, int cap_a)
{
    const int cap_s0 = (corr_rows + 127) / 128 * 128;
    return cap_s0 < cap_a ? cap_s0 : cap_a;
}

size_t carve_lazy(void *base, LazyWs &w, int B, int C, int cap_a, int cap_q, int S, int corr_rows)
{
    Carver carve(base, carve_screen8_raw(base, w, B, C, cap_a, cap_q, S));
    const size_t rows = (size_t)B * cap_a, pairs = (size_t)B;
    carve(w.margin, rows);
    carve(w.sid_final, rows);
    carve(w.unc_idx, rows);
    carve(w.state, rows);
    carve(w.sel_rows, pairs * corr_rows);
    carve(w.scratch, rows);
    carve(w.n_a_eager, pairs);
    carve(w.n_a_lazy, pairs);
    carve(w.ambu_idx, rows);
    carve(w.ambv_idx, pairs * corr_rows);
    const size_t cap_s = sampled_cap(corr_rows, cap_a);
    const size_t e1 = oryon_match_workspace_bytes(B, cap_a), e2 = oryon_match_workspace_bytes(B, (int)cap_s);
    w.exact_ws_bytes = e1 > e2 ? e1 : e2;
    carve(w.exact_ws, w.exact_ws_bytes > 16 ? w.exact_ws_bytes : 16);
    carve(w.x3_ah, pairs * cap_s * C);
    carve(w.x3_al, pairs * cap_s * C);
    carve(w.x3_a_ovf, pairs * cap_s * C);
    carve(w.x3_md_o, pairs * cap_s);
    carve(w.x3_am_o, pairs * cap_s);
    carve(w.x3_va_o, pairs * cap_s);
    carve(w.x3_scratch, match_x3_scratch_bytes(B, (int)cap_s, 8, cap_q));
    const bool cascade = C == 256 && corr_rows <= MX6_SAMPLED_PANEL;
    const size_t triples = cascade ? pairs * mx6_sampled_splits(B) * MX6_SAMPLED_PANEL : 4;
    carve(w.cs_panel, cascade ? pairs * MX6_SAMPLED_PANEL * C : 16);
    if (!cascade) w.cs_panel = nullptr;
    carve(w.cs_max, triples);
    carve(w.cs_m2, triples);
    carve(w.cs_i1, triples);
    carve(w.n_ambv0, pairs);
    carve(w.cs_gate, pairs * mx6_panels_per_pair(cap_a));
    w.lazy_zero_off = carve.off;
    carve(w.pair_eager, pairs);
    carve(w.n_unc, pairs);
    carve(w.n_ambu, pairs);
    carve(w.n_ambv, pairs);
    carve(w.need_f32_lazy, pairs);
    carve(w.n_amb_total, pairs);
    carve(w.mark, rows);
    w.lazy_zero_bytes = carve.off - w.lazy_zero_off;
    return carve.off;
}
}

extern "C" size_t oryon_match_corrs_i8_workspace_bytes(int B, int C, int cap_a, int cap_q, int corr_rows)
{
    if (B <= 0 || C <= 0 || cap_a <= 0 || cap_a % MT16 || cap_q <= 0 || corr_rows <= 0) return 0;
    LazyWs w;
    return carve_lazy(nullptr, w, B, C, cap_a, cap_q, pick_split16(B, cap_a / MT16), corr_rows);
}

namespace {
constexpr const char *IMPL = "match_corrs_lazy_impl";

int select_step(const MatchCorrsArgs &m, const LazyWs &w, hipStream_t st)
{
    const int rc = select_corrs_launch(m.roi_a, m.roi_q, m.roi_stride_a, m.roi_stride_q, m.n_a, m.n_q, m.argmin, m.valid, m.cap_a, m.B, m.W,
                                       m.max_corrs, m.corr_rows, m.seed, m.pair_key, w.scratch, m.corrs, m.n_valid, m.n_sel, m.status,
                                       w.sel_rows, w.pair_eager, st);
    if (rc) set_error("oryon_match_corrs_i8: select launch failed");
    return rc;
}

int eager_route(const MatchCorrsArgs &m, const LazyWs &w, int S)
{
    decide8_step(m, S, w.n_a_eager, w);
    rescore_raw_step(m, w.n_a_eager, 2, w);
    int rc = check_launch(IMPL);
    if (rc) return rc;
    if ((rc = raw_fallbacks(m, w.n_a_eager, w, IMPL, "oryon_match_corrs_i8"))) return rc;
    return select_step(m, w, as_stream(m.stream));
}

void compact_anchors(const MatchCorrsArgs &m, const AnchorRaw &araw, const LazyWs &w, hipStream_t st, int cap_c, const int32_t *count,
                     const int32_t *idx, int idx_stride)
{
    const dim3 grid((cap_c + 63) / 64, m.B);
    if (m.a_hat)
        hipLaunchKernelGGL(match_compact_f32_kernel, grid, dim3(256), 0, st, m.a_hat, m.C, m.cap_a, cap_c, count, idx, idx_stride, w.a_hat_c);
    else
        hipLaunchKernelGGL(m.layout == ORYON_LAYOUT_NHWC ? match_compact_raw_kernel<true> : match_compact_raw_kernel<false>, grid, dim3(256), 0,
                           st, araw, m.C_true, m.HW, m.round_f16, m.C, m.cap_a, cap_c, count, idx, idx_stride, w.a_hat_c);
}

int lazy_route(const MatchCorrsArgs &m, const LazyWs &w, hipStream_t st, int use_x3, bool cascade)
{
    const int B = m.B, C = m.C, cap_a = m.cap_a, cap_q = m.cap_q, corr_rows = m.corr_rows;
    const bool nhwc = m.layout == ORYON_LAYOUT_NHWC;
    const AnchorRaw araw = {m.feat_a, m.roi_a, m.a_norm, m.roi_stride_a};
    int rc = gather_q8_launch(m.feat_q, B, m.C_true, m.HW, m.layout, m.roi_q, m.roi_stride_q, m.n_q, w.need_f32_lazy, cap_q, C, w.q8_scratch,
                              w.scale_scratch, w.eps_scratch, nullptr, w.q_hat, 1, m.round_f16, st);
    if (rc) { set_error("oryon_match_corrs_i8: lazy fp32 gather launch failed"); return rc; }
    compact_anchors(m, araw, w, st, cap_a, w.n_ambu, w.ambu_idx, cap_a);
    if ((rc = check_launch(IMPL))) return rc;
    rc = oryon_match_f32(w.a_hat_c, w.q_hat, B, C, cap_a, cap_q, w.n_ambu, m.n_q, m.threshold, w.md_c, w.am_c, w.va_c, w.exact_ws,
                         w.exact_ws_bytes, st);
    if (rc) return rc;
    hipLaunchKernelGGL(match_scatter_exact_kernel, dim3(cap_a / 256, B), dim3(256), 0, st, cap_a, cap_a, w.n_ambu, w.ambu_idx, cap_a, w.md_c,
                       w.am_c, w.va_c, m.min_dist, m.argmin, m.valid, w.state);
    if ((rc = check_launch(IMPL))) return rc;
    const size_t lds_res = (size_t)4 * 2 * C * sizeof(float);
    auto resolve_uncertain = m.fmt == 1 ? (nhwc ? match_resolve_uncertain_kernel<true, 1> : match_resolve_uncertain_kernel<false, 1>)
                                        : (nhwc ? match_resolve_uncertain_kernel<true, 0> : match_resolve_uncertain_kernel<false, 0>);
    hipLaunchKernelGGL(resolve_uncertain, dim3(64, B), dim3(256), lds_res, st, m.a_hat, araw, m.a_i8, m.q_i8, m.q_scale, m.a_scale, m.feat_q,
                       m.C_true, m.HW, m.roi_q, m.roi_stride_q, m.q_norm, C, cap_a, cap_q, m.n_q, m.threshold, w.m_final, w.sid_final, w.margin,
                       w.n_unc, w.unc_idx, w.pair_eager, w.state, m.valid, m.min_dist, m.argmin, m.round_f16);
    if ((rc = check_launch(IMPL))) return rc;
    if ((rc = select_step(m, w, st))) return rc;
    const int cap_s = sampled_cap(corr_rows, cap_a);
    hipLaunchKernelGGL(match_list_sampled_amb_kernel, dim3(B), dim3(256), 0, st, cap_a, w.state, w.pair_eager, m.n_sel, w.sel_rows, corr_rows,
                       w.mark, w.n_ambv, w.ambv_idx);
    if (cascade) {
        const int csS = mx6_sampled_splits(B);
        hipLaunchKernelGGL(match_compact_rows_kernel, dim3(MX6_SAMPLED_PANEL / 16, B), dim3(256), 0, st, reinterpret_cast<const uint8_t *>(m.a_i8),
                           C, cap_a, MX6_SAMPLED_PANEL, w.n_ambv, w.ambv_idx, corr_rows, w.cs_panel);
        launch_screen_mx6_sampled(st, w.cs_panel, reinterpret_cast<const uint8_t *>(m.q_i8), B, cap_q, w.n_ambv, m.n_q, csS, w.cs_max, w.cs_i1,
                                  w.cs_m2, m.C_true);
        hipLaunchKernelGGL(match_decide_sampled_kernel, dim3((MX6_SAMPLED_PANEL + 255) / 256, B), dim3(256), 0, st, cap_a, MX6_SAMPLED_PANEL, csS,
                           w.n_ambv, w.ambv_idx, corr_rows, w.cs_max, w.cs_i1, w.cs_m2, m.a_scale, m.q_eps_max, w.m_final, w.sid_final,
                           w.margin, w.state, w.mark, w.n_ambv0);
        hipLaunchKernelGGL(match_list_sampled_amb_kernel, dim3(B), dim3(256), 0, st, cap_a, w.state, w.pair_eager, m.n_sel, w.sel_rows,
                           corr_rows, w.mark, w.n_ambv, w.ambv_idx);
        if ((rc = check_launch(IMPL))) return rc;
    }
    compact_anchors(m, araw, w, st, cap_s, w.n_ambv, w.ambv_idx, corr_rows);
    if ((rc = check_launch(IMPL))) return rc;
    if (use_x3) {
        __half *qh = reinterpret_cast<__half *>(w.q_hat), *ql = qh + (size_t)B * cap_q * C;
        int32_t *n_ovf = nullptr, *ovf_idx = nullptr;
        rc = match_x3_resolve(w.a_hat_c, w.n_ambv, cap_s, m.feat_q, m.C_true, m.HW, m.layout, m.roi_q, m.roi_stride_q, m.q_norm, m.n_q, B, cap_q,
                              m.threshold, m.round_f16, qh, ql, w.x3_ah, w.x3_al, w.x3_scratch, w.md_c, w.am_c, w.va_c, &n_ovf, &ovf_idx,
                              w.ambv_idx, corr_rows, w.sid_final, cap_a, static_cast<const __half *>(m.q_hi_lo), m.q_lo_sq_max, st);
        if (rc) { set_error("oryon_match_corrs: fp16x3 second-level launch failed"); return rc; }
        rc = gather_q8_launch(m.feat_q, B, m.C_true, m.HW, m.layout, m.roi_q, m.roi_stride_q, m.n_q, n_ovf, cap_q, C, w.q8_scratch,
                              w.scale_scratch, w.eps_scratch, nullptr, w.q_hat, 1, m.round_f16, st);
        if (rc) { set_error("oryon_match_corrs: overflow fp32 gather launch failed"); return rc; }
        hipLaunchKernelGGL(match_compact_f32_kernel, dim3((cap_s + 63) / 64, B), dim3(256), 0, st, w.a_hat_c, C, cap_s, cap_s, n_ovf, ovf_idx,
                           cap_s, w.x3_a_ovf);
        if ((rc = check_launch(IMPL))) return rc;
        rc = oryon_match_f32(w.x3_a_ovf, w.q_hat, B, C, cap_s, cap_q, n_ovf, m.n_q, m.threshold, w.x3_md_o, w.x3_am_o, w.x3_va_o, w.exact_ws,
                             w.exact_ws_bytes, st);
        if (rc) return rc;
        match_x3_scatter_ovf(B, cap_s, n_ovf, ovf_idx, w.x3_md_o, w.x3_am_o, w.x3_va_o, w.md_c, w.am_c, w.va_c, st);
    } else {
        rc = oryon_match_f32(w.a_hat_c, w.q_hat, B, C, cap_s, cap_q, w.n_ambv, m.n_q, m.threshold, w.md_c, w.am_c, w.va_c, w.exact_ws,
                             w.exact_ws_bytes, st);
        if (rc) return rc;
    }
    hipLaunchKernelGGL(match_scatter_exact_kernel, dim3((cap_s + 255) / 256, B), dim3(256), 0, st, cap_a, cap_s, w.n_ambv, w.ambv_idx,
                       corr_rows, w.md_c, w.am_c, w.va_c, m.min_dist, m.argmin, m.valid, w.state);
    if ((rc = check_launch(IMPL))) return rc;
    auto resolve_selected = m.fmt == 1 ? (nhwc ? match_resolve_selected_kernel<true, 1> : match_resolve_selected_kernel<false, 1>)
                                       : (nhwc ? match_resolve_selected_kernel<true, 0> : match_resolve_selected_kernel<false, 0>);
    hipLaunchKernelGGL(resolve_selected, dim3((m.max_corrs + 3) / 4, B), dim3(256), lds_res, st, m.a_hat, araw, m.a_i8, m.q_i8, m.q_scale,
                       m.a_scale, m.feat_q, m.C_true, m.HW, m.roi_q, m.roi_stride_q, m.q_norm, C, cap_a, cap_q, m.n_q, m.W, w.m_final,
                       w.sid_final, w.margin, w.state, w.pair_eager, m.n_sel, w.sel_rows, corr_rows, m.min_dist, m.argmin, m.corrs,
                       m.round_f16);
    if ((rc = check_launch(IMPL))) return rc;
    if (m.n_undecided && cascade) {
        hipLaunchKernelGGL(match_cascade_counts_kernel, dim3((B + 255) / 256), dim3(256), 0, st, B, w.n_amb_total, w.n_ambv, w.n_ambv0,
                           m.n_undecided);
        if ((rc = check_launch(IMPL))) return rc;
    } else if (m.n_undecided) {
        hipLaunchKernelGGL(match_sum_counts_kernel, dim3((B + 255) / 256), dim3(256), 0, st, B, w.n_amb, w.n_amb_total, m.n_undecided);
        if ((rc = check_launch(IMPL))) return rc;
    }
    return ORYON_OK;
}
}

int oryon::match_corrs_lazy_impl(const MatchCorrsArgs &m)
{
    ORYON_CHECK_ARG((m.a_hat || (m.feat_a && m.a_norm && !m.force_eager)) && m.a_i8 && m.a_scale && m.feat_q && m.roi_a && m.roi_q && m.q_norm && m.q_i8 && m.q_eps_max && m.n_a && m.n_q);
    ORYON_CHECK_ARG((m.fmt == 0 || m.fmt == 1) && (m.fmt == 1 || m.q_scale) && !(m.fmt == 1 && m.force_eager));
    ORYON_CHECK_ARG(!m.q_hi_lo || (m.q_lo_sq_max && m.C == 256));
    ORYON_CHECK_ARG(m.min_dist && m.argmin && m.valid && m.corrs && m.n_valid && m.n_sel && m.status);
    ORYON_CHECK_ARG(m.B >= 0 && (m.C == 256 || m.C == 512) && m.C_true > 0 && m.C_true <= m.C && m.HW > 0 && m.W > 0 && m.max_corrs > 0 && m.corr_rows >= m.max_corrs);
    ORYON_CHECK_ARG(m.layout == ORYON_LAYOUT_NCHW || m.layout == ORYON_LAYOUT_NHWC);
    ORYON_CHECK_ARG(m.cap_a > 0 && m.cap_a % MT16 == 0 && m.cap_q > 0 && m.cap_q % 256 == 0 && m.threshold > 0.0f && m.threshold <= 0.5f);
    if (m.B == 0) return ORYON_OK;
    const int B = m.B, C = m.C, cap_a = m.cap_a, cap_q = m.cap_q;
    const int T = cap_a / MT16;
    const int S = pick_split16(B, T);
    LazyWs w;
    const size_t need = carve_lazy(m.workspace, w, B, C, cap_a, cap_q, S, m.corr_rows);
    if (!m.workspace || m.workspace_bytes < need) {
        set_error("oryon_match_corrs_i8: workspace too small (%zu < %zu)", m.workspace_bytes, need);
        return ORYON_ERR_WORKSPACE;
    }
    hipStream_t st = as_stream(m.stream);
    ORYON_CHECK_HIP(hipMemsetAsync(static_cast<char *>(m.workspace) + w.zero_off, 0, w.zero_bytes, st));
    if (m.force_eager) ORYON_CHECK_HIP(hipMemsetAsync(w.need_f32, 0, (size_t)B * sizeof(int32_t), st));
    ORYON_CHECK_HIP(hipMemsetAsync(static_cast<char *>(m.workspace) + w.lazy_zero_off, 0, w.lazy_zero_bytes, st));
    const float cut0 = 1.0f - 2.0f * m.threshold;
    static const bool x3_env = dev_env_int("ORYON_AMB_X3", 1) != 0;
    const int use_x3 = (x3_env && C == 256 && !m.force_eager) ? 1 : 0;
    static const bool cascade_env = dev_env_int("ORYON_CASCADE", 1) != 0;
    const bool cascade = cascade_env && m.fmt == 1 && use_x3 && m.q_hi_lo != nullptr && w.cs_panel != nullptr;
    if (m.fmt == 1) {
        const uint8_t *a6 = reinterpret_cast<const uint8_t *>(m.a_i8), *q6 = reinterpret_cast<const uint8_t *>(m.q_i8);
        const int groups = ((B * S + 7) / 8) * 8 * T;
        profile_begin(st, screen_mx6_name(C));
        if (cascade) {
            const int T8 = mx6_panels_per_pair(cap_a);
            launch_screen_mx6(C, groups, T, st, a6, q6, B, cap_a, cap_q, m.n_a, m.n_q, S, w.ws_max, w.ws_i1, w.ws_m2, m.C_true, 1, nullptr, 2);
            hipLaunchKernelGGL(match_panel_settle_kernel, dim3(T8, B), dim3(256), 0, st, cap_a, T8, S, m.n_a, w.ws_max, w.ws_m2, m.a_scale,
                               m.q_eps_max, cut0, w.cs_gate);
            launch_screen_mx6(C, groups, T, st, a6, q6, B, cap_a, cap_q, m.n_a, m.n_q, S, w.ws_max, w.ws_i1, w.ws_m2, m.C_true, 1, w.cs_gate, 0);
        } else {
            launch_screen_mx6(C, groups, T, st, a6, q6, B, cap_a, cap_q, m.n_a, m.n_q, S, w.ws_max, w.ws_i1, w.ws_m2, m.C_true);
        }
        profile_end(st);
    } else {
        screen8_step(m, S, m.n_a, w);
    }
    ORYON_CHECK_LAUNCH();
    hipLaunchKernelGGL(match_decide_lite_kernel, dim3(cap_a / 256, B), dim3(256), 0, st, cap_a, m.n_a, S, w.ws_max, w.ws_i1, w.ws_m2, m.a_scale,
                       m.q_eps_max, cut0, sqrtf((float)m.C_true), (float)m.C_true, m.force_eager, m.fmt, use_x3, w.m_final, w.sid_final, w.margin,
                       w.state, m.valid, m.min_dist, m.argmin, w.pair_eager, w.n_unc, w.unc_idx, w.n_ambu, w.ambu_idx, w.need_f32_lazy,
                       w.n_amb_total);
    hipLaunchKernelGGL(match_mask_counts_kernel, dim3((B + 255) / 256), dim3(256), 0, st, B, m.n_a, w.pair_eager, w.n_a_eager, w.n_a_lazy);
    ORYON_CHECK_LAUNCH();
    if (!m.force_eager) return lazy_route(m, w, st, use_x3, cascade);
    const int rc = eager_route(m, w, S);
    if (rc) return rc;
    if (m.n_undecided) ORYON_CHECK_HIP(hipMemcpyAsync(m.n_undecided, w.n_amb, (size_t)B * sizeof(int32_t), hipMemcpyDeviceToDevice, st));
    return ORYON_OK;
}

namespace {
MatchCorrsArgs shared_args(const float *feat_q, int C_true, int HW, int layout, const int32_t *roi_a, int roi_stride_a, const int32_t *roi_q,
                           int roi_stride_q, const float *q_norm, int B, int C, int cap_a, int cap_q, const int32_t *n_a, const int32_t *n_q,
                           float threshold, int W, int max_corrs, int corr_rows, uint64_t seed, const int64_t *pair_key, float *min_dist,
                           int32_t *argmin, uint8_t *valid, int32_t *corrs, int32_t *n_valid, int32_t *n_sel, int32_t *status,
                           int32_t *n_undecided, int round_f16, void *workspace, size_t workspace_bytes, void *stream)
{
    MatchCorrsArgs m;
    m.feat_q = feat_q;
    m.C_true = C_true;
    m.HW = HW;
    m.layout = layout;
    m.roi_a = roi_a;
    m.roi_stride_a = roi_stride_a;
    m.roi_q = roi_q;
    m.roi_stride_q = roi_stride_q;
    m.q_norm = q_norm;
    m.B = B;
    m.C = C;
    m.cap_a = cap_a;
    m.cap_q = cap_q;
    m.n_a = n_a;
    m.n_q = n_q;
    m.threshold = threshold;
    m.W = W;
    m.max_corrs = max_corrs;
    m.corr_rows = corr_rows;
    m.seed = seed;
    m.pair_key = pair_key;
    m.min_dist = min_dist;
    m.argmin = argmin;
    m.valid = valid;
    m.corrs = corrs;
    m.n_valid = n_valid;
    m.n_sel = n_sel;
    m.status = status;
    m.n_undecided = n_undecided;
    m.round_f16 = round_f16;
    m.workspace = workspace;
    m.workspace_bytes = workspace_bytes;
    m.stream = stream;
    return m;
}
}

extern "C" int oryon_match_corrs_i8(const float *a_hat, const int8_t *a_i8, const float *a_scale, const float *feat_q, int C_true, int HW,
                                    int layout, const int32_t *roi_a, int roi_stride_a, const int32_t *roi_q, int roi_stride_q,
                                    const float *q_norm, const int8_t *q_i8, const float *q_scale, const float *q_eps_max, int B, int C,
                                    int cap_a, int cap_q, const int32_t *n_a, const int32_t *n_q, float threshold, int W, int max_corrs,
                                    int corr_rows, uint64_t seed, const int64_t *pair_key, int force_eager, float *min_dist,
                                    int32_t *argmin, uint8_t *valid, int32_t *corrs, int32_t *n_valid, int32_t *n_sel, int32_t *status,
                                    int32_t *n_undecided, int round_f16, void *workspace, size_t workspace_bytes, void *stream)
{
    ORYON_CHECK_ARG(a_scale && q_scale);
    MatchCorrsArgs m = shared_args(feat_q, C_true, HW, layout, roi_a, roi_stride_a, roi_q, roi_stride_q, q_norm, B, C, cap_a, cap_q, n_a, n_q,
                                   threshold, W, max_corrs, corr_rows, seed, pair_key, min_dist, argmin, valid, corrs, n_valid, n_sel, status,
                                   n_undecided, round_f16, workspace, workspace_bytes, stream);
    m.a_hat = a_hat;
    m.a_i8 = a_i8;
    m.a_scale = a_scale;
    m.q_i8 = q_i8;
    m.q_scale = q_scale;
    m.q_eps_max = q_eps_max;
    m.force_eager = force_eager;
    return match_corrs_lazy_impl(m);
}

extern "C" int oryon_match_corrs_mx6(const float *a_hat, const uint8_t *a_mx6, const float *a_err_max, const float *feat_q, int C_true, int HW,
                                     int layout, const int32_t *roi_a, int roi_stride_a, const int32_t *roi_q, int roi_stride_q,
                                     const float *q_norm, const uint8_t *q_mx6, const float *q_err_max, int B, int C, int cap_a, int cap_q,
                                     const int32_t *n_a, const int32_t *n_q, float threshold, int W, int max_corrs, int corr_rows,
                                     uint64_t seed, const int64_t *pair_key, float *min_dist, int32_t *argmin, uint8_t *valid,
                                     int32_t *corrs, int32_t *n_valid, int32_t *n_sel, int32_t *status, int32_t *n_undecided, int round_f16,
                                     void *workspace, size_t workspace_bytes, void *stream)
{
    ORYON_CHECK_ARG(a_err_max && q_err_max);
    MatchCorrsArgs m = shared_args(feat_q, C_true, HW, layout, roi_a, roi_stride_a, roi_q, roi_stride_q, q_norm, B, C, cap_a, cap_q, n_a, n_q,
// ... 104 lines not shown
```

oryon_amd/csrc/screen_mx6.hip:

```cpp
#include <hip/hip_runtime.h>
#include <stdio.h>
#include <stdlib.h>
#include <type_traits>
#include "common.h"
#include "match_common.h"

namespace oryon {

typedef int i32x4 __attribute__((ext_vector_type(4)));
constexpr int screen8_tile_bytes(int CP) { return CP * 128; }

typedef int i32x8 __attribute__((ext_vector_type(8)));
typedef float f32x16s __attribute__((ext_vector_type(16)));

template <int CP, int WAVES = 8, int VAR = 0>
__global__ __launch_bounds__(64 * WAVES, CP == 512 ? 1 : 2) void match_mx6_screen_kernel(
    const uint8_t *__restrict__ a6, const uint8_t *__restrict__ q6, int B, int cap_a, int cap_q, const int32_t *__restrict__ n_a,
    const int32_t *__restrict__ n_q, int T, int S, float *__restrict__ ws_max, int32_t *__restrict__ ws_i1, float *__restrict__ ws_m2)
{
    constexpr int RB = CP;
    constexpr int TILE_BYTES = screen8_tile_bytes(CP);
    constexpr int ROWS = 128, NQB = 4, NAB = 2;
    constexpr int NKS = CP / 64;
    constexpr int NI = TILE_BYTES / (1024 * WAVES);
// ... 275 lines not shown
    f32x16s acc[NAB];
#pragma unroll
    for (int ab = 0; ab < NAB; ++ab)
#pragma unroll
        for (int r = 0; r < 16; ++r) acc[ab][r] = -3.0e38f;
    int sid01 = 0, sid23 = 0;

    auto mfma = [&](f32x16s &d, int ab, auto SC) {
        constexpr int s_ = decltype(SC)::value;
        d = __builtin_amdgcn_mfma_scale_f32_32x32x64_f8f6f4(areg[s_], breg[ab][s_], s_ == 0 ? zero16 : d, 2, 2, 0, areg[s_][6], s_ & 3,
                                                            bsc[ab][s_ >> 2]);
    };
    int buf = 0;
    for (int qt = qt_begin; qt < qt_end; ++qt) {
        const unsigned tile = buf * TILE_BYTES;
        const int qt_next = qt + 1 < qt_end ? qt + 1 : qt;
#pragma unroll
        for (int qb = 0; qb < NQB; ++qb) {
            const int sid = (qt * NQB + qb) * 2 + hi;
            if (qb == 0) {
#pragma unroll
                for (int j = 0; j < NI; ++j) issue_one(qt_next, buf ^ 1, j);
            }
            reduce_block(acc[2], sid23, 2);
            reduce_block(acc[3], sid23, 3);
            mx6_static_for<0, KL>([&](auto SC) { mfma(acc[0], 0, SC); mfma(acc[1], 1, SC); });
#pragma unroll
            for (int i = 0; i < 2 * KL; ++i) {
                __builtin_amdgcn_sched_group_barrier(0x008, 1, 0);
                __builtin_amdgcn_sched_group_barrier(0x002, 16 / KL, 0);
            }
            mx6_static_for<0, KL>([&](auto SC) {
                constexpr int s_ = decltype(SC)::value;
                mfma(acc[2], 2, SC); mfma(acc[3], 3, SC);
                if (qb + 1 < NQB) areg[s_] = rd(s_, qb + 1, tile);
            });
            reduce_block(acc[0], sid, 0);
            reduce_block(acc[1], sid, 1);
#pragma unroll
            for (int i = 0; i < 2 * KL; ++i) {
                __builtin_amdgcn_sched_group_barrier(0x008, 1, 0);
                __builtin_amdgcn_sched_group_barrier(0x002, 16 / KL, 0);
                if (qb + 1 < NQB && (i & 1)) __builtin_amdgcn_sched_group_barrier(0x100, 2, 0);
            }
            sid01 = sid;
            sid23 = sid;
        }
        asm volatile("s_waitcnt vmcnt(0)" ::: "memory");
        __syncthreads();
        buf ^= 1;
#pragma unroll
        for (int s = 0; s < KL; ++s) areg[s] = rd(s, 0, buf * TILE_BYTES);
    }
    (void)sid01;
    reduce_block(acc[2], sid23, 2);
    reduce_block(acc[3], sid23, 3);
#pragma unroll
    for (int ab = 0; ab < NAB; ++ab) {
        const float om1 = __shfl_xor(runmax[ab], 32), om2 = __shfl_xor(run2[ab], 32);
        const int oi1 = __shfl_xor(runidx[ab], 32);
        const float m1 = fmaxf(runmax[ab], om1);
        const float m2 = fmaxf(fminf(runmax[ab], om1), fmaxf(run2[ab], om2));
        const int i1 = (om1 > runmax[ab]) ? oi1 : runidx[ab];
        const int a = a0 + wave * (32 * NAB) + ab * 32 + l31;
        if (hi == 0 && a < cap_a) {
            const size_t o = ((size_t)p * S + split) * cap_a + a;
            ws_max[o] = m1;
            ws_i1[o] = i1;
            ws_m2[o] = m2;
        }
    }
    if (dbg_wg && t == 0) {
        dbg_wg[(size_t)blockIdx.x * 4 + 0] = tk0;
        dbg_wg[(size_t)blockIdx.x * 4 + 1] = wall_clock64();
        dbg_wg[(size_t)blockIdx.x * 4 + 2] = (long long)__builtin_amdgcn_s_getreg((31 << 11) | 4);
        dbg_wg[(size_t)blockIdx.x * 4 + 3] = (long long)__builtin_amdgcn_s_getreg((31 << 11) | 20);
    }
}

template <int CP, int WAVES, int KL = CP / 64>
__global__ __launch_bounds__(64 * WAVES, CP == 512 ? 1 : 2) void match_mx6_screen_w4_win_kernel(
    const uint8_t *__restrict__ a6, const uint8_t *__restrict__ q6, int B, int cap_a, int cap_q, const int32_t *__restrict__ n_a,
    const int32_t *__restrict__ n_q, int T, int S, float *__restrict__ ws_max, int32_t *__restrict__ ws_i1, float *__restrict__ ws_m2,
    const int32_t *__restrict__ gate , int win )
{
    static_assert(CP == 256 || (CP == 512 && WAVES == 4), "geometries: C_pad 256 with 4 / 8 waves, C_pad 512 with 4 waves");
    constexpr int RB = CP, NAB = 4;
    constexpr int TILE_BYTES = screen8_tile_bytes(CP);
    constexpr int ROWS = 128, NQB = 4;
    constexpr int NKS = CP / 64;
    constexpr int NI = TILE_BYTES / (1024 * WAVES);
    constexpr int LPR = RB / 256;
    char *smem;
    if constexpr (2 * TILE_BYTES > 65536) {
        extern __shared__ __attribute__((aligned(256))) char smem_dyn_w4w[];
        smem = smem_dyn_w4w;
    } else {
        __shared__ __attribute__((aligned(256))) char smem_st_w4w[2 * TILE_BYTES];
        smem = smem_st_w4w;
    }
    const int xcd = blockIdx.x & 7, slot = blockIdx.x >> 3;
    const int unit = (slot / T) * 8 + xcd;
    if (unit >= B * S) return;
    const int panel = slot % T;
    const int p = unit / S, split = unit % S;
    const int na = n_a[p], nq = n_q[p];
    const int a0 = panel * (32 * NAB * WAVES);
    if (a0 >= na) return;
    if (gate && gate[p * T + panel] == 0) return;
    const int nqt = (nq + ROWS - 1) / ROWS;
    const int qt_per = (nqt + S - 1) / S;
    int qt_begin = split * qt_per;
    int qt_end = (qt_begin + qt_per < nqt) ? qt_begin + qt_per : nqt;
    if (win > 0 && qt_end - qt_begin > win) {
        const int cnt = qt_end - qt_begin, panels = (na + 32 * NAB * WAVES - 1) / (32 * NAB * WAVES);
        int k0 = (int)(((long long)(2 * panel + 1) * cnt) / (2 * panels)) - win / 2;
        k0 = k0 < 0 ? 0 : (k0 > cnt - win ? cnt - win : k0);
        qt_begin += k0;
        qt_end = qt_begin + win;
    }
    const int t = threadIdx.x, lane = t & 63, wave = t >> 6, l31 = lane & 31, hi = lane >> 5;
    const char *qp = reinterpret_cast<const char *>(q6) + (size_t)p * cap_q * RB;

    i32x8 breg[NAB][NKS];
    int bsc[NAB][NKS / 4];
#pragma unroll
    for (int ab = 0; ab < NAB; ++ab) {
        const int arow_i = a0 + wave * (32 * NAB) + ab * 32 + l31;
        const char *arow = reinterpret_cast<const char *>(a6) + ((size_t)p * cap_a + (arow_i < cap_a ? arow_i : cap_a - 1)) * RB + 32 * hi;
        unsigned sc[NKS / 4];
#pragma unroll
        for (int w = 0; w < NKS / 4; ++w) sc[w] = 0;
#pragma unroll
        for (int s = 0; s < KL; ++s) {
            const i32x4 lo = *reinterpret_cast<const i32x4 *>(arow + 64 * s), up = *reinterpret_cast<const i32x4 *>(arow + 64 * s + 16);
            breg[ab][s] = __builtin_shufflevector(lo, up, 0, 1, 2, 3, 4, 5, -1, -1);
            sc[s >> 2] |= ((unsigned)up[2] & 0xffu) << (8 * (s & 3));
        }
#pragma unroll
        for (int w = 0; w < NKS / 4; ++w) bsc[ab][w] = (int)sc[w];
    }
    constexpr int DJ = 4 * LPR;
    static_assert(NI % DJ == 0 || NI == DJ, "DMA instructions per wave and tile");
    unsigned dma_off[DJ];
#pragma unroll
    for (int j = 0; j < DJ; ++j) {
        const int line = (wave * NI + j) * 4 + (lane >> 4), sl = lane & 15;
        const int row = line / LPR;
        dma_off[j] = (unsigned)(row * RB + (((line % LPR) * 16 + (sl ^ (row & 15))) << 4));
    }
    const int wave_u = __builtin_amdgcn_readfirstlane(wave);
    auto issue_one = [&](int qt, int buf, int j) {
        const char *qb = qp + (size_t)qt * TILE_BYTES + (j / DJ) * (16 * RB);
        char *dst = smem + buf * TILE_BYTES + (wave_u * NI + j) * 1024;
        __builtin_amdgcn_global_load_lds((const __attribute__((address_space(1))) void *)(qb + dma_off[j % DJ]),
                                         (__attribute__((address_space(3))) void *)dst, 16, 0, 0);
    };
    unsigned koff[4][2];
#pragma unroll
    for (int c = 0; c < 4; ++c)
#pragma unroll
        for (int e = 0; e < 2; ++e) koff[c][e] = (unsigned)(l31 * RB) + ((((unsigned)(4 * c + 2 * hi + e)) ^ (unsigned)(l31 & 15)) << 4);
    auto rd = [&](int s, int qb, unsigned tile) -> i32x8 {
        const unsigned base = tile + (unsigned)(qb * 32 * RB + (s >> 2) * 256);
        const i32x4 lo = *reinterpret_cast<const i32x4 *>(smem + koff[s & 3][0] + base);
        const i32x4 up = *reinterpret_cast<const i32x4 *>(smem + koff[s & 3][1] + base);
        return __builtin_shufflevector(lo, up, 0, 1, 2, 3, 4, 5, 6, -1);
    };

    float runmax[NAB], run2[NAB];
    int runidx[NAB];
#pragma unroll
    for (int ab = 0; ab < NAB; ++ab) { runmax[ab] = -INFINITY; run2[ab] = -INFINITY; runidx[ab] = 0; }
    auto reduce_block = [&](const f32x16s &c, int sid, int ab) {
        const float m0 = fmaxf(fmaxf(c[0], c[1]), c[2]), m1 = fmaxf(fmaxf(c[3], c[4]), c[5]), m2 = fmaxf(fmaxf(c[6], c[7]), c[8]);
        const float m3 = fmaxf(fmaxf(c[9], c[10]), c[11]), m4 = fmaxf(fmaxf(c[12], c[13]), c[14]);
        const float x = fmaxf(fmaxf(fmaxf(m0, m1), m2), fmaxf(fmaxf(m3, m4), c[15]));
        const bool improved = x > runmax[ab];
        run2[ab] = __builtin_amdgcn_fmed3f(runmax[ab], run2[ab], x);
        runmax[ab] = __builtin_amdgcn_fmed3f(runmax[ab], x, INFINITY);
        runidx[ab] = improved ? sid : runidx[ab];
    };
    const f32x16s zero16 = {0, 0, 0, 0, 0, 0, 0, 0, 0, 0, 0, 0, 0, 0, 0, 0};

    if (qt_end > qt_begin) {
#pragma unroll
        for (int j = 0; j < NI; ++j) issue_one(qt_begin, 0, j);
    }
    asm volatile("s_waitcnt vmcnt(0)" ::: "memory");
    __syncthreads();

    i32x8 areg[NKS];
#pragma unroll
    for (int s = 0; s < KL; ++s) areg[s] = rd(s, 0, 0u);
    f32x16s acc[NAB];
#pragma unroll
    for (int ab = 0; ab < NAB; ++ab)
#pragma unroll
        for (int r = 0; r < 16; ++r) acc[ab][r] = -3.0e38f;
    int sid01 = 0, sid23 = 0;

    auto mfma = [&](f32x16s &d, int ab, auto SC) {
        constexpr int s_ = decltype(SC)::value;
// ... 21 lines not shown
            }
            mx6_static_for<0, KL>([&](auto SC) {
                constexpr int s_ = decltype(SC)::value;
                mfma(acc[2], 2, SC); mfma(acc[3], 3, SC);
                if (qb + 1 < NQB) areg[s_] = rd(s_, qb + 1, tile);
            });
            reduce_block(acc[0], sid, 0);
            reduce_block(acc[1], sid, 1);
#pragma unroll
            for (int i = 0; i < 2 * KL; ++i) {
                __builtin_amdgcn_sched_group_barrier(0x008, 1, 0);
                __builtin_amdgcn_sched_group_barrier(0x002, 16 / KL, 0);
                if (qb + 1 < NQB && (i & 1)) __builtin_amdgcn_sched_group_barrier(0x100, 2, 0);
            }
            sid01 = sid;
            sid23 = sid;
        }
        asm volatile("s_waitcnt vmcnt(0)" ::: "memory");
        __syncthreads();
        buf ^= 1;
#pragma unroll
        for (int s = 0; s < KL; ++s) areg[s] = rd(s, 0, buf * TILE_BYTES);
    }
    (void)sid01;
    reduce_block(acc[2], sid23, 2);
    reduce_block(acc[3], sid23, 3);
#pragma unroll
    for (int ab = 0; ab < NAB; ++ab) {
        const float om1 = __shfl_xor(runmax[ab], 32), om2 = __shfl_xor(run2[ab], 32);
        const int oi1 = __shfl_xor(runidx[ab], 32);
        const float m1 = fmaxf(runmax[ab], om1);
        const float m2 = fmaxf(fminf(runmax[ab], om1), fmaxf(run2[ab], om2));
        const int i1 = (om1 > runmax[ab]) ? oi1 : runidx[ab];
        const int a = a0 + wave * (32 * NAB) + ab * 32 + l31;
        if (hi == 0 && a < cap_a) {
            const size_t o = ((size_t)p * S + split) * cap_a + a;
            ws_max[o] = m1;
            ws_i1[o] = i1;
            ws_m2[o] = m2;
        }
    }
}

static void mx6_debug_report(const long long *dbg_dev, int groups, hipStream_t st)
{
    (void)hipStreamSynchronize(st);
    long long *w = static_cast<long long *>(malloc((size_t)groups * 4 * sizeof(long long)));
    (void)hipMemcpy(w, dbg_dev, (size_t)groups * 4 * sizeof(long long), hipMemcpyDeviceToHost);
    long long t0 = -1, t1 = 0;
    double sum = 0;
    int ran = 0;
    long long longest = 0;
    for (int g = 0; g < groups; ++g)
        if (w[4 * g + 1]) {
            if (t0 < 0 || w[4 * g] < t0) t0 = w[4 * g];
            if (w[4 * g + 1] > t1) t1 = w[4 * g + 1];
            sum += (double)(w[4 * g + 1] - w[4 * g]);
            if (w[4 * g + 1] - w[4 * g] > longest) longest = w[4 * g + 1] - w[4 * g];
            ++ran;
        }
    fprintf(stderr, "[mx6] %d of %d workgroups ran: span %.1f us, mean %.1f us, longest %.1f us, mean residency %.1f workgroups\n", ran, groups,
            (t1 - t0) * 0.01, ran ? sum * 0.01 / ran : 0.0, longest * 0.01, t1 > t0 ? sum / (double)(t1 - t0) : 0.0);
    fprintf(stderr, "[mx6] resident at 5%%..95%% of the span:");
    for (int k = 0; k < 10; ++k) {
        const long long ts = t0 + (t1 - t0) * (2 * k + 1) / 20;
        int r = 0;
        for (int g = 0; g < groups; ++g) r += w[4 * g + 1] && w[4 * g] <= ts && ts < w[4 * g + 1];
        fprintf(stderr, " %d", r);
    }
    fprintf(stderr, "\n");
    free(w);
}

static int mx6_var()
{
    static const int var = dev_env_int("ORYON_MX6_VAR", 0);
    return var;
}

namespace {
template <int CP>
void launch_screen_mx6_t(int groups, int T, hipStream_t st, const uint8_t *a6, const uint8_t *q6, int B, int cap_a, int cap_q, const int32_t *n_a,
                       const int32_t *n_q, int S, float *ws_max, int32_t *ws_i1, float *ws_m2, int kl = 0, bool gate_or_win = false,
                       const int32_t *gate = nullptr, int win = 0)
{
    constexpr size_t dyn = 2 * screen8_tile_bytes(CP) > 65536 ? 2 * screen8_tile_bytes(CP) : 0;
    constexpr int W_ = CP == 512 ? 4 : 8;
    const int Tw = (cap_a + 64 * W_ - 1) / (64 * W_);
    const int var = mx6_var();
    if (var == 1) {
        if (dyn) allow_dynamic_lds(reinterpret_cast<const void *>(&match_mx6_screen_kernel<CP, W_, 1>), (int)dyn);
        hipLaunchKernelGGL((match_mx6_screen_kernel<CP, W_, 1>), dim3(groups / T * Tw), dim3(64 * W_), dyn, st, a6, q6, B, cap_a, cap_q, n_a, n_q, Tw,
                           S, ws_max, ws_i1, ws_m2);
        return;
    }
    if constexpr (CP == 256) {
        if (var == 0) {
            const int T8 = (cap_a + 1023) / 1024;
            static const bool dbg = dev_env_set("ORYON_MX6_DEBUG");
            static long long *dbg_wg = nullptr;
            const int g8 = groups / T * T8;
            if (dbg && !dbg_wg) (void)hipMalloc(&dbg_wg, (size_t)65536 * 4 * sizeof(long long));
            if (dbg && dbg_wg && g8 <= 65536) (void)hipMemsetAsync(dbg_wg, 0, (size_t)g8 * 4 * sizeof(long long), st);
            if (gate_or_win) {
#define ORYON_LAUNCH_WIN(KLV)                                                                                                         \
    hipLaunchKernelGGL((match_mx6_screen_w4_win_kernel<CP, 8, KLV>), dim3(g8), dim3(512), 0, st, a6, q6, B, cap_a, cap_q, n_a, n_q, T8, S,   \
                       ws_max, ws_i1, ws_m2, gate, win)
                if (kl == 1) ORYON_LAUNCH_WIN(1);
                else if (kl == 2) ORYON_LAUNCH_WIN(2);
                else ORYON_LAUNCH_WIN(4);
#undef ORYON_LAUNCH_WIN
                return;
            }
            if (kl == 1)
                hipLaunchKernelGGL((match_mx6_screen_w4_kernel<CP, 8, 1>), dim3(g8), dim3(512), 0, st, a6, q6, B, cap_a, cap_q, n_a, n_q, T8, S,
                                   ws_max, ws_i1, ws_m2, (dbg && g8 <= 65536) ? dbg_wg : nullptr);
            else if (kl == 2)
                hipLaunchKernelGGL((match_mx6_screen_w4_kernel<CP, 8, 2>), dim3(g8), dim3(512), 0, st, a6, q6, B, cap_a, cap_q, n_a, n_q, T8, S,
                                   ws_max, ws_i1, ws_m2, (dbg && g8 <= 65536) ? dbg_wg : nullptr);
            else
            hipLaunchKernelGGL((match_mx6_screen_w4_kernel<CP, 8>), dim3(g8), dim3(512), 0, st, a6, q6, B, cap_a, cap_q, n_a, n_q, T8, S,
                               ws_max, ws_i1, ws_m2, (dbg && g8 <= 65536) ? dbg_wg : nullptr);
            if (dbg && dbg_wg && g8 <= 65536) mx6_debug_report(dbg_wg, g8, st);
            return;
        }
        if (var == 3) {
            hipLaunchKernelGGL((match_mx6_screen_w4_kernel<CP, 4>), dim3(groups / T * Tw), dim3(256), 0, st, a6, q6, B, cap_a, cap_q, n_a, n_q, Tw, S,
                               ws_max, ws_i1, ws_m2, nullptr);
            return;
        }
    }
    if constexpr (CP == 512) {
        if (var == 0) {
            allow_dynamic_lds(reinterpret_cast<const void *>(&match_mx6_screen_w4_kernel<CP, 4>), (int)dyn);
            hipLaunchKernelGGL((match_mx6_screen_w4_kernel<CP, 4>), dim3(groups / T * Tw), dim3(256), dyn, st, a6, q6, B, cap_a, cap_q, n_a, n_q, Tw,
                               S, ws_max, ws_i1, ws_m2, nullptr);
            return;
        }
    }
    if (dyn) allow_dynamic_lds(reinterpret_cast<const void *>(&match_mx6_screen_kernel<CP, W_>), (int)dyn);
    hipLaunchKernelGGL((match_mx6_screen_kernel<CP, W_>), dim3(groups / T * Tw), dim3(64 * W_), dyn, st, a6, q6, B, cap_a, cap_q, n_a, n_q, Tw, S,
                       ws_max, ws_i1, ws_m2);
}
}

const char *screen_mx6_name(int C)
{
    if (C != 256) return mx6_var() == 0 ? "match_mx6_screen_w4_kernel<512, 4>" : "match_mx6_screen_kernel<512, 4, 0>";
    return mx6_var() == 0 ? "match_mx6_screen_w4_kernel<256, 8>" : mx6_var() == 3 ? "match_mx6_screen_w4_kernel<256, 4>" : mx6_var() == 1 ? "match_mx6_screen_kernel<256, 8, 1>" : "match_mx6_screen_kernel<256, 8, 0>";
}

void launch_screen_mx6(int C, int groups, int T, hipStream_t st, const uint8_t *a6, const uint8_t *q6, int B, int cap_a, int cap_q,
                       const int32_t *n_a, const int32_t *n_q, int S, float *ws_max, int32_t *ws_i1, float *ws_m2, int C_true,
                       int cascade, const int32_t *gate, int win)
{
    const int kl = (C == 256 && C_true > 0 && C_true <= 64) ? 1 : (C == 256 && C_true > 0 && C_true <= 128) ? 2 : 0;
    if (C == 256) launch_screen_mx6_t<256>(groups, T, st, a6, q6, B, cap_a, cap_q, n_a, n_q, S, ws_max, ws_i1, ws_m2, kl, cascade != 0, gate, win);
    else launch_screen_mx6_t<512>(groups, T, st, a6, q6, B, cap_a, cap_q, n_a, n_q, S, ws_max, ws_i1, ws_m2);
}

void launch_screen_mx6_sampled(hipStream_t st, const uint8_t *a6_panel, const uint8_t *q6, int B, int cap_q, const int32_t *n_rows,
                               const int32_t *n_q, int S, float *ws_max, int32_t *ws_i1, float *ws_m2, int C_true)
{
    const int groups = ((B * S + 7) / 8) * 8;
    const int kl = (C_true > 0 && C_true <= 64) ? 1 : (C_true > 0 && C_true <= 128) ? 2 : 0;
    if (kl == 1)
        hipLaunchKernelGGL((match_mx6_screen_w4_kernel<256, 4, 1>), dim3(groups), dim3(256), 0, st, a6_panel, q6, B, 512, cap_q, n_rows, n_q, 1, S,
                           ws_max, ws_i1, ws_m2, static_cast<long long *>(nullptr));
    else if (kl == 2)
        hipLaunchKernelGGL((match_mx6_screen_w4_kernel<256, 4, 2>), dim3(groups), dim3(256), 0, st, a6_panel, q6, B, 512, cap_q, n_rows, n_q, 1, S,
                           ws_max, ws_i1, ws_m2, static_cast<long long *>(nullptr));
    else
        hipLaunchKernelGGL((match_mx6_screen_w4_kernel<256, 4>), dim3(groups), dim3(256), 0, st, a6_panel, q6, B, 512, cap_q, n_rows, n_q, 1, S,
                           ws_max, ws_i1, ws_m2, static_cast<long long *>(nullptr));
}

}
```

oryon_amd/engine.py:

```python
from __future__ import annotations

import ctypes
from dataclasses import dataclass, field
from typing import Dict, Optional, Tuple

import torch
from torch import Tensor

from . import _lib, ops
from ._lib import check, lib
from .pointdsc import PointDSC

PAIR_OK, PAIR_NO_MASK, PAIR_NO_CORR = 0, 1, 2
SOLVERS = ("pointdsc", "ransac")
_default_solver = "pointdsc"


def set_default_solver(name: str) -> None:
    global _default_solver
    if name not in SOLVERS:
        raise ValueError(f"Solver {name} not implemented")
    _default_solver = name


def default_solver() -> str:
    return _default_solver


@dataclass
class MatchPoseConfig:
    dist_th: float = 0.25
    n_corrs: int = 500
    src_sampling: Optional[int] = 5000
    seed: int = 1
    match_mode: str = "screened"
    half_descriptors: bool = False
    sample_first: int = 0
    solver: str = field(default_factory=default_solver)
    ransac_max_iter: int = 10000
    ransac_match_err: float = 0.001
    ransac_fix_percent: float = 0.9999


def _check_solver(cfg: "MatchPoseConfig", solver) -> bool:
    if cfg.solver not in SOLVERS:
        raise ValueError(f"Solver {cfg.solver} not implemented")
    if cfg.solver == "pointdsc" and solver is None:
        raise ValueError("solver='pointdsc' needs a PointDSC model")
    return cfg.solver == "ransac"


def _cfg_sig(cfg: "MatchPoseConfig", overlap: int) -> Tuple:
    return (cfg.dist_th, cfg.n_corrs, cfg.src_sampling, cfg.seed, cfg.half_descriptors, overlap, int(cfg.sample_first), cfg.solver,
            cfg.ransac_max_iter, cfg.ransac_match_err, cfg.ransac_fix_percent)


class NativeStep:

    _SLOT_VIEWS = {
        "pose": (torch.float32, lambda g: (g["B"], 4, 4)), "status_out": (torch.int32, lambda g: (g["B"],)),
        "n_valid": (torch.int32, lambda g: (g["B"],)), "n_lift": (torch.int32, lambda g: (g["B"],)),
        "n_valid_out": (torch.int32, lambda g: (g["B"],)), "n_lift_out": (torch.int32, lambda g: (g["B"],)),
        "n_a": (torch.int32, lambda g: (g["B"],)), "n_q": (torch.int32, lambda g: (g["B"],)), "n_und": (torch.int32, lambda g: (g["B"],)),
        "n_sel": (torch.int32, lambda g: (g["B"],)), "status": (torch.int32, lambda g: (g["B"],)),
        "roi_a": (torch.int32, lambda g: (g["B"], g["HW"])), "roi_q": (torch.int32, lambda g: (g["B"], g["HW"])),
        "min_dist": (torch.float32, lambda g: (g["B"], g["cap_a"])), "argmin": (torch.int32, lambda g: (g["B"], g["cap_a"])),
        "valid": (torch.uint8, lambda g: (g["B"], g["cap_a"])), "corrs": (torch.int32, lambda g: (g["B"], g["n_cap"], 4)),
        "pcd_a": (torch.float32, lambda g: (g["B"], g["n_cap"], 3)), "pcd_q": (torch.float32, lambda g: (g["B"], g["n_cap"], 3)),
    }

    def __init__(self, solver: Optional[PointDSC], cfg: "MatchPoseConfig", key: Tuple, dev: torch.device, overlap: int, n_slots: int = 6,
                 gather_sets: int = 2, reg_streams: int = 2, reg_lag: int = 0, screen: int = 1, x3_prefetch: int = 1,
                 stream_roles: int = 0):
        B, C, FH, FW, HA, WA, HQ, WQ, layout = key
        self.key, self.dev = key, dev
        if overlap >= 2:
            from . import configure
            configure()
        ransac = _check_solver(cfg, solver)
        if not ransac:
            solver._ensure_handle(dev)
        self._solver = solver
        handle = None if ransac else solver._handle
        self.ecfg = _lib.EngineConfig(B=B, C=C, FH=FH, FW=FW, HA=HA, WA=WA, HQ=HQ, WQ=WQ, layout=layout, dist_th=cfg.dist_th,
                                      n_corrs=cfg.n_corrs, src_sampling=int(cfg.src_sampling or 0), seed=int(cfg.seed) & (2**64 - 1),
                                      round_f16=int(cfg.half_descriptors), n_slots=n_slots, overlap=overlap,
                                      gather_sets=min(gather_sets, n_slots), reg_streams=reg_streams,
                                      reg_lag=reg_lag if overlap else 0, screen=screen,
                                      sample_first=int(cfg.sample_first) if cfg.sample_first and cfg.sample_first > 0 else 0,
                                      x3_prefetch=int(bool(x3_prefetch)) if (C <= 256 and screen == 1) else 0,
                                      stream_roles=int(stream_roles), solver=int(ransac), ransac_max_iter=int(cfg.ransac_max_iter),
                                      ransac_match_err=float(cfg.ransac_match_err), ransac_fix_percent=float(cfg.ransac_fix_percent))
        self.cfg_sig = _cfg_sig(cfg, overlap)
        need = lib().oryon_engine_arena_bytes(ctypes.byref(self.ecfg), handle)
        if need == 0:
            raise _lib.OryonError(f"oryon_engine_arena_bytes: {lib().oryon_last_error().decode()}")
        with torch.cuda.device(dev):
            self.arena = torch.empty((need,), dtype=torch.uint8, device=dev)
            self._h = ctypes.c_void_p()
            check(lib().oryon_engine_create(ctypes.byref(self._h), ctypes.byref(self.ecfg), handle, self.arena.data_ptr(), need),
                  "oryon_engine_create")
        ca, cq, cp, nc = ctypes.c_int(), ctypes.c_int(), ctypes.c_int(), ctypes.c_int()
        check(lib().oryon_engine_geometry(self._h, ctypes.byref(ca), ctypes.byref(cq), ctypes.byref(cp), ctypes.byref(nc)))
        self.geo = dict(B=B, HW=FH * FW, cap_a=ca.value, cap_q=cq.value, c_pad=cp.value, n_cap=nc.value)
        self.n_slots = n_slots
        self.steps = 0
        self._views = [dict() for _ in range(n_slots)]
        self.reads_pending = [None] * n_slots

    def __del__(self):
        try:
            if getattr(self, "_h", None):
                torch.cuda.synchronize(self.dev)
                lib().oryon_engine_destroy(self._h)
                self._h = None
        except Exception:
            pass

    def view(self, slot: int, name: str) -> Tensor:
        v = self._views[slot].get(name)
        if v is None:
            off, nbytes = ctypes.c_size_t(), ctypes.c_size_t()
            check(lib().oryon_engine_buffer(self._h, slot, name.encode(), ctypes.byref(off), ctypes.byref(nbytes)), "oryon_engine_buffer")
            dtype, shape = self._SLOT_VIEWS[name]
            v = self.arena[off.value: off.value + nbytes.value].view(dtype).view(shape(self.geo))
            self._views[slot][name] = v
        return v

    def set_timing(self, on: bool) -> None:
        check(lib().oryon_engine_set_timing(self._h, int(on)))

    def stream_roles(self) -> int:
        r = ctypes.c_int()
        check(lib().oryon_engine_stream_roles(self._h, ctypes.byref(r)))
        return r.value

    def set_stream_roles(self, roles: int) -> None:
        with torch.cuda.device(self.dev):
            check(lib().oryon_engine_set_stream_roles(self._h, int(roles)), "oryon_engine_set_stream_roles")

    def timing(self, step: int) -> Dict[str, float]:
        out = (ctypes.c_float * 8)()
        check(lib().oryon_engine_timing(self._h, int(step), out), "oryon_engine_timing")
        names = ("gather_ms", "match_ms", "screen_kernel_ms", "registration_ms", "match_start", "match_end", "registration_start",
                 "registration_end")
        return dict(zip(names, (float(x) for x in out)))

    def elapsed(self, step_a: int, event_a: int, step_b: int, event_b: int) -> float:
        ms = ctypes.c_float()
        check(lib().oryon_engine_elapsed(self._h, int(step_a), event_a, int(step_b), event_b, ctypes.byref(ms)), "oryon_engine_elapsed")
        return float(ms.value)

    def gather_ms(self, step: int) -> float:
        ms = ctypes.c_float()
        check(lib().oryon_engine_gather_ms(self._h, int(step), ctypes.byref(ms)), "oryon_engine_gather_ms")
        return float(ms.value)

    def x3_steps(self) -> int:
        n = ctypes.c_int64()
        check(lib().oryon_engine_x3_steps(self._h, ctypes.byref(n)))
        return n.value

    def feedback(self) -> Optional[Tuple[int, int, int]]:
        st, und, na = ctypes.c_int64(), ctypes.c_int64(), ctypes.c_int64()
        check(lib().oryon_engine_feedback(self._h, ctypes.byref(st), ctypes.byref(und), ctypes.byref(na)))
        return None if st.value < 0 else (st.value, und.value, na.value)

    def host_stats(self) -> Tuple[int, float, float]:
        n, tot, last = ctypes.c_int64(), ctypes.c_double(), ctypes.c_double()
        check(lib().oryon_engine_host_stats(self._h, ctypes.byref(n), ctypes.byref(tot), ctypes.byref(last)))
        return n.value, tot.value, last.value

    def submit(self, feat_a, feat_q, mask_a, mask_q, depth_a, depth_q, cam_a, cam_q, pair_key, force_eager: bool, inputs_resident: bool) -> int:
        with torch.cuda.device(self.dev):
            slot = lib().oryon_engine_submit(self._h, feat_a.data_ptr(), feat_q.data_ptr(), mask_a.data_ptr(), mask_q.data_ptr(),
                                             depth_a.data_ptr(), depth_q.data_ptr(), cam_a.data_ptr(), cam_q.data_ptr(),
                                             None if pair_key is None else pair_key.data_ptr(), int(force_eager), int(inputs_resident),
                                             torch.cuda.current_stream(self.dev).cuda_stream)
        if slot < 0:
            check(slot, "oryon_engine_submit")
        self.steps += 1
        return slot

    def next_slot(self) -> int:
        return self.steps % self.n_slots

    def wait(self, slot: int) -> None:
        check(lib().oryon_engine_wait(self._h, slot, torch.cuda.current_stream(self.dev).cuda_stream), "oryon_engine_wait")


class MatchPoseEngine:
    def __init__(self, solver: Optional[PointDSC], cfg: Optional[MatchPoseConfig] = None, overlap_registration: bool = False,
                 overlap_gather: bool = False, native: bool = True, result_views: bool = False):
        self.solver = solver
        self.cfg = cfg or MatchPoseConfig()
        _check_solver(self.cfg, solver)
        self.n_cap = ops.round_up(self.cfg.n_corrs, 128)
        self.overlap = overlap_registration
        self.overlap_gather = overlap_gather
        self.native = native
        self.result_views = result_views
        self._native: Optional[NativeStep] = None
        self._inflight: Dict[int, Dict[str, Tensor]] = {}
        self.native_geometry = dict(n_slots=6, gather_sets=2, reg_streams=2, reg_lag=0, screen=1, x3_prefetch=1, stream_roles=0)
        self.native_timing = False
        self._reg_stream = None
        self.reg_streams = 2
        self._gather_stream = None
        self.i8_max_undecided = 2.0
        self.collect_i8_stats = False
        self.i8_retry_every = 16
        self._i8_pending = None
        self._i8_host = None
        self._i8_frac = 0.0
        self._i8_skipped = 0

    DEFAULT_ROLES = 2345
    ROLE_CANDIDATES = (2345, 6345, 2341, 6341, 2301)

    def tune_stream_roles(self, run_steps, candidates: Optional[Tuple[int, ...]] = None, steps: int = 8, warm: int = 2) -> Dict[str, object]:
        import time
        nat = self._native
        if nat is None or nat.ecfg.overlap == 0:
            return {"roles": None, "ms_per_step": {}, "default": self.DEFAULT_ROLES}
        cands = tuple(candidates or self.ROLE_CANDIDATES)
        seen: Dict[int, float] = {}
        for r in cands:
            nat.set_stream_roles(r)
            run_steps(warm)
            torch.cuda.synchronize(nat.dev)
            t0 = time.perf_counter()
            run_steps(steps)
            torch.cuda.synchronize(nat.dev)
            seen[r] = (time.perf_counter() - t0) / steps * 1e3
        best = min(seen, key=seen.get)
        if self.DEFAULT_ROLES in seen and seen[self.DEFAULT_ROLES] <= seen[best] * 1.01:
            best = self.DEFAULT_ROLES
        nat.set_stream_roles(best)
        self.native_geometry["stream_roles"] = best
        return {"roles": best, "ms_per_step": {str(k): round(v, 4) for k, v in seen.items()}, "default": self.DEFAULT_ROLES}

    def finish(self, out: Dict[str, Tensor]) -> Dict[str, Tensor]:
        slot = out.pop("_native_slot", None)
        if slot is not None:
            self._native.wait(slot)
            out.pop("_inputs", None)
            queued = False
            if self.collect_i8_stats or self.i8_max_undecided < 1.0:
                fb = self._native.feedback() if len(out) <= 4 else None
                if fb is not None and fb[2] > 0:
                    self._i8_frac = fb[1] / fb[2]
                elif self._i8_pending is None and (len(out) > 4 or self._native.ecfg.screen != 1):
                    self._queue_i8_stats(self._native.view(slot, "n_und"), self._native.view(slot, "n_a"))
                    queued = True
            if not self.result_views:
                for k, v in list(out.items()):
                    if isinstance(v, Tensor):
                        out[k] = v.clone()
                queued = queued or len(out) > 4
            elif len(out) > 4:
                self._native.reads_pending[slot] = True
            if queued and self._native.reads_pending[slot] is not True:
                ev = torch.cuda.Event()
                ev.record(torch.cuda.current_stream(self._native.dev))
                self._native.reads_pending[slot] = ev
            if self._inflight.get(slot) is out:
                del self._inflight[slot]
            return out
        ev = out.pop("_done", None)
        if ev is not None:
            cur = torch.cuda.current_stream(out["pose"].device)
            cur.wait_event(ev)
            for k in ("pose", "status"):
                out[k].record_stream(cur)
        return out

    def _py_mark(self, idx: int, stream) -> None:
        tl = getattr(self, "py_timeline", None)
        if tl is None:
            return
        if idx == 0:
            tl.append({})
        ev = torch.cuda.Event(enable_timing=True)
        ev.record(stream)
        tl[-1][idx] = ev

    def _queue_i8_stats(self, n_und: Tensor, n_a: Tensor) -> None:
# ... 223 lines not shown
```

Baseline: 19910.

## Add probe-driven band cascade to skip distant query tiles in mx6 screening

Adds a default-on screening cascade for C=256. It first screens a strided sample of anchor rows against all query tiles, then derives a per-panel band of query tiles around the confident nearest neighbours. The full screen runs only over that band. Rows whose best score clears an error-bounded sure line are settled, and the remaining open rows are compacted for exact follow-up. The goal is to cut the dominant match screening work, at the cost of extra probe, settle and scatter kernels, more workspace, and correctness that depends on the error-bound heuristic. A cascade-stats query is also exposed for inspection.

```diff
diff --git a/include/oryon_hip.h b/include/oryon_hip.h
--- a/include/oryon_hip.h
+++ b/include/oryon_hip.h
@@ -247,6 +247,7 @@
     int sample_first;
     int x3_prefetch;
     int stream_roles;
+    int screen_cascade;
     int solver;
     int ransac_max_iter;
     float ransac_match_err;
@@ -272,6 +273,7 @@
 int oryon_engine_gather_ms(oryon_engine_t *handle, int64_t step, float *ms);
 int oryon_engine_host_stats(const oryon_engine_t *handle, int64_t *n_submit, double *submit_ms_total, double *submit_ms_last);
 int oryon_engine_x3_steps(const oryon_engine_t *handle, int64_t *n_steps);
+int oryon_engine_cascade_stats(oryon_engine_t *handle, int32_t *out);
 int oryon_engine_feedback(oryon_engine_t *handle, int64_t *step, int64_t *n_undecided, int64_t *n_anchors);
 
 int oryon_split_f16x3(const float *x, int64_t n, void *hi_f16, void *lo_f16, void *stream);
diff --git a/oryon_amd/_lib.py b/oryon_amd/_lib.py
--- a/oryon_amd/_lib.py
+++ b/oryon_amd/_lib.py
@@ -18,7 +18,7 @@
 class EngineConfig(ctypes.Structure):
     _fields_ = [("B", c_int), ("C", c_int), ("FH", c_int), ("FW", c_int), ("HA", c_int), ("WA", c_int), ("HQ", c_int), ("WQ", c_int),
                 ("layout", c_int), ("dist_th", c_float), ("n_corrs", c_int), ("src_sampling", c_int), ("seed", c_uint64),
-                ("round_f16", c_int), ("n_slots", c_int), ("overlap", c_int), ("gather_sets", c_int), ("reg_streams", c_int), ("reg_lag", c_int), ("screen", c_int), ("sample_first", c_int), ("x3_prefetch", c_int), ("stream_roles", c_int),
+                ("round_f16", c_int), ("n_slots", c_int), ("overlap", c_int), ("gather_sets", c_int), ("reg_streams", c_int), ("reg_lag", c_int), ("screen", c_int), ("sample_first", c_int), ("x3_prefetch", c_int), ("stream_roles", c_int), ("screen_cascade", c_int),
                 ("solver", c_int), ("ransac_max_iter", c_int), ("ransac_match_err", c_float), ("ransac_fix_percent", c_float)]
 
 
@@ -133,6 +133,7 @@
     "oryon_engine_config_bytes": (c_size_t, []),
     "oryon_engine_host_stats": (c_int, [c_void_p, POINTER(c_int64), POINTER(ctypes.c_double), POINTER(ctypes.c_double)]),
     "oryon_engine_x3_steps": (c_int, [c_void_p, POINTER(c_int64)]),
+    "oryon_engine_cascade_stats": (c_int, [c_void_p, c_void_p]),
     "oryon_engine_feedback": (c_int, [_P, POINTER(c_int64), POINTER(c_int64), POINTER(c_int64)]),
     "oryon_fusion_window_attention_f32": (c_int, [_P, _P, c_int, c_int, c_int, c_int, c_int, c_int, c_int, _P, _P]),
     "oryon_fusion_class_layer_f32": (c_int, [_P, _P, POINTER(FusionClassWeights), c_int, _P, _P]),
diff --git a/oryon_amd/csrc/engine.hip b/oryon_amd/csrc/engine.hip
--- a/oryon_amd/csrc/engine.hip
+++ b/oryon_amd/csrc/engine.hip
@@ -2,6 +2,7 @@
 #include <chrono>
 #include <new>
 #include <vector>
+#include <string.h>
 #include "common.h"
 #include "match_common.h"
 
@@ -203,7 +204,7 @@
     ORYON_CHECK_ARG((c->layout == ORYON_LAYOUT_NCHW || c->layout == ORYON_LAYOUT_NHWC) && (c->screen == 0 || c->screen == 1));
     ORYON_CHECK_ARG(c->overlap >= 0 && c->overlap <= 2 && (c->overlap == 0 || c->n_slots >= 2));
     ORYON_CHECK_ARG((size_t)c->C * (size_t)c->FH * (size_t)c->FW * 4u < (1ull << 32));
-    ORYON_CHECK_ARG(c->sample_first >= 0 && (c->x3_prefetch == 0 || c->x3_prefetch == 1));
+    ORYON_CHECK_ARG(c->sample_first >= 0 && (c->x3_prefetch == 0 || c->x3_prefetch == 1) && (c->screen_cascade == 0 || c->screen_cascade == 1));
     ORYON_CHECK_ARG(roles_valid(c->stream_roles));
     ORYON_CHECK_ARG(c->solver == 0 || (c->solver == 1 && c->ransac_max_iter > 0 && c->ransac_match_err >= 0.0f));
     return ORYON_OK;
@@ -563,6 +564,7 @@
         m.workspace_bytes = e->L.match_ws_bytes;
         m.stream = sm;
         m.fmt = mx6 ? 1 : 0;
+        m.cascade = (c.screen_cascade && !sf) ? 1 : 0;
         if (mx6 && x3_pre) {
             m.a_hat = g.a_hat;
             m.q_hi_lo = g.q_hilo;
@@ -667,6 +669,16 @@
     return ORYON_OK;
 }
 
+extern "C" int oryon_engine_cascade_stats(oryon_engine_t *e, int32_t *out)
+{
+    ORYON_CHECK_ARG(e && out);
+    ORYON_CHECK_HIP(hipDeviceSynchronize());
+    const int32_t *stats = match_dc_stats(e->L.match_ws, e->cfg.B, e->L.c_pad, e->L.cap_a, e->L.cap_q, e->L.n_cap);
+    if (!stats) { memset(out, 0, (size_t)e->cfg.B * 4 * sizeof(int32_t)); return ORYON_OK; }
+    ORYON_CHECK_HIP(hipMemcpy(out, stats, (size_t)e->cfg.B * 4 * sizeof(int32_t), hipMemcpyDeviceToHost));
+    return ORYON_OK;
+}
+
 extern "C" int oryon_engine_timing(oryon_engine_t *e, int64_t step, float *out8)
 {
     ORYON_CHECK_ARG(e && out8 && step >= 0 && step < e->n_submit && step >= e->n_submit - TIMING_RING);
diff --git a/oryon_amd/csrc/match_common.h b/oryon_amd/csrc/match_common.h
--- a/oryon_amd/csrc/match_common.h
+++ b/oryon_amd/csrc/match_common.h
@@ -30,9 +30,11 @@
 const char *screen_mx6_name(int C);
 void launch_screen_mx6(int C, int groups, int T, hipStream_t st, const uint8_t *a6, const uint8_t *q6, int B, int cap_a, int cap_q,
                        const int32_t *n_a, const int32_t *n_q, int S, float *ws_max, int32_t *ws_i1, float *ws_m2, int C_true,
-                       int cascade = 0, const int32_t *gate = nullptr, int win = 0);
+                       int cascade = 0, const int32_t *gate = nullptr, int win = 0, const int32_t *band = nullptr);
 inline int mx6_panels_per_pair(int cap_a) { return (cap_a + 1023) / 1024; }
 void launch_screen_mx6_sampled(hipStream_t st, const uint8_t *a6_panel, const uint8_t *q6, int B, int cap_q, const int32_t *n_rows,
+                               const int32_t *n_q, int S, float *ws_max, int32_t *ws_i1, float *ws_m2, int C_true);
+void launch_screen_mx6_rows512(hipStream_t st, const uint8_t *a6_rows, const uint8_t *q6, int B, int cap_rows, int cap_q, const int32_t *n_rows,
                                const int32_t *n_q, int S, float *ws_max, int32_t *ws_i1, float *ws_m2, int C_true);
 constexpr int MX6_SAMPLED_PANEL = 512;
 inline int mx6_sampled_splits(int B) { int s = (512 + B - 1) / B; return s < 1 ? 1 : s > 16 ? 16 : s; }
@@ -142,7 +144,9 @@
     size_t workspace_bytes = 0;
     int fmt = 0;
     int force_eager = 0;
+    int cascade = 1;
 };
 int match_corrs_lazy_impl(const MatchCorrsArgs &m);
+int32_t *match_dc_stats(void *workspace, int B, int C, int cap_a, int cap_q, int corr_rows);
 
 }
diff --git a/oryon_amd/csrc/match_corrs.hip b/oryon_amd/csrc/match_corrs.hip
--- a/oryon_amd/csrc/match_corrs.hip
+++ b/oryon_amd/csrc/match_corrs.hip
@@ -191,11 +191,12 @@
 
 __global__ __launch_bounds__(256) void match_compact_rows_kernel(const uint8_t *__restrict__ rows, int row_bytes, int cap_a, int cap_c,
                                                                   const int32_t *__restrict__ count, const int32_t *__restrict__ idx,
-                                                                  int idx_stride, uint8_t *__restrict__ out)
+                                                                  int idx_stride, uint8_t *__restrict__ out, int fill_mult)
 {
     const int p = blockIdx.y, sl = blockIdx.x * 16 + (threadIdx.x >> 4), l = threadIdx.x & 15;
     if (sl >= cap_c) return;
     const int n = count[p] < cap_c ? count[p] : cap_c;
+    if (sl >= (n + fill_mult - 1) / fill_mult * fill_mult) return;
     uint4 *d = reinterpret_cast<uint4 *>(out + ((size_t)p * cap_c + sl) * row_bytes);
     if (sl >= n) {
         for (int i = l; i < row_bytes / 16; i += 16) d[i] = make_uint4(0, 0, 0, 0);
@@ -212,7 +213,7 @@
                                                                     const float *__restrict__ q_err, float *__restrict__ m_final,
                                                                     int32_t *__restrict__ sid_final, float *__restrict__ margin_out,
                                                                     uint8_t *__restrict__ state, int32_t *__restrict__ mark,
-                                                                    int32_t *__restrict__ count_before)
+                                                                    int32_t *__restrict__ count_before, float *__restrict__ min_dist)
 {
     const int p = blockIdx.y, sl = blockIdx.x * 256 + threadIdx.x;
     const int n = count[p] < cap_c ? count[p] : cap_c;
@@ -234,10 +235,163 @@
     m_final[arow] = m1;
     sid_final[arow] = sid;
     margin_out[arow] = margin;
+    if (min_dist) min_dist[arow] = __fmaf_rn(-0.5f, m1, 0.5f);
     if (m1 - m2 > margin) {
         state[arow] = LZ_VALID;
         mark[arow] = 0;
     }
+}
+
+constexpr uint8_t DC_COMPLETE = 0, DC_SETTLED = 1, DC_OPEN = 2;
+constexpr int DC_SLACK = 2;
+constexpr int DC_MIN_SURE = 8;
+constexpr int DC_BAND_CAP_NUM = 1, DC_BAND_CAP_DEN = 2;
+
+__device__ __forceinline__ float dc_sure_line(const float *__restrict__ a_err, const float *__restrict__ q_err, int p, float cut0)
+{
+    const float ea = a_err[p], eq = q_err[p];
+    const float delta = ea + eq + ea * eq + 1.2e-4f;
+    return delta < 0.2f ? cut0 + delta + 2e-5f : INFINITY;
+}
+
+__device__ __forceinline__ void dc_merge(const float *__restrict__ ws_m1, const int32_t *__restrict__ ws_i1, const float *__restrict__ ws_m2,
+                                         int p, int S, int cap, int r, float &m1, int &sid, float &m2)
+{
+    m1 = -INFINITY;
+    m2 = -INFINITY;
+    sid = 0;
+    for (int s = 0; s < S; ++s) {
+        const size_t o = ((size_t)p * S + s) * cap + r;
+        const float x1 = ws_m1[o], x2 = ws_m2[o];
+        m2 = fmaxf(fminf(m1, x1), fmaxf(m2, x2));
+        if (x1 > m1) { m1 = x1; sid = ws_i1[o]; }
+    }
+}
+
+__global__ __launch_bounds__(256) void match_dc_probe_list_kernel(int stride, const int32_t *__restrict__ n_a, int32_t *__restrict__ n_probe,
+                                                                   int32_t *__restrict__ probe_idx)
+{
+    const int p = blockIdx.x;
+    int n = (n_a[p] + stride - 1) / stride;
+    n = n < MX6_SAMPLED_PANEL ? n : MX6_SAMPLED_PANEL;
+    for (int k = threadIdx.x; k < n; k += 256) probe_idx[(size_t)p * MX6_SAMPLED_PANEL + k] = k * stride;
+    if (threadIdx.x == 0) n_probe[p] = n;
+}
+
+__global__ __launch_bounds__(256) void match_dc_probe_band_kernel(int cap_a, int T8, int stride, int S, const int32_t *__restrict__ n_a,
+                                                                   const int32_t *__restrict__ n_q, const float *__restrict__ cs_m1,
+                                                                   const int32_t *__restrict__ cs_i1, const float *__restrict__ cs_m2,
+                                                                   const float *__restrict__ a_err, const float *__restrict__ q_err, float cut0,
+                                                                   float *__restrict__ r_m1, int32_t *__restrict__ r_i1, float *__restrict__ r_m2,
+                                                                   int32_t *__restrict__ band, int32_t *__restrict__ stats, int slack)
+{
+    __shared__ int lo, hi, cnt;
+    const int p = blockIdx.y, panel = blockIdx.x, t = threadIdx.x;
+    const int na = n_a[p], a0 = panel * 1024;
+    if (a0 >= na) return;
+    if (t == 0) { lo = 0x7fffffff; hi = -1; cnt = 0; }
+    __syncthreads();
+    const int a1 = a0 + 1024 < na ? a0 + 1024 : na;
+    const int k_lo = (a0 + stride - 1) / stride;
+    int k_hi = (a1 + stride - 1) / stride;
+    k_hi = k_hi < MX6_SAMPLED_PANEL ? k_hi : MX6_SAMPLED_PANEL;
+    const float line = dc_sure_line(a_err, q_err, p, cut0);
+    for (int k = k_lo + t; k < k_hi; k += 256) {
+        float m1, m2;
+        int sid;
+        dc_merge(cs_m1, cs_i1, cs_m2, p, S, MX6_SAMPLED_PANEL, k, m1, sid, m2);
+        const size_t arow = (size_t)p * cap_a + (size_t)k * stride;
+        r_m1[arow] = m1;
+        r_i1[arow] = sid;
+        r_m2[arow] = m2;
+        if (m1 > line) {
+            atomicMin(&lo, sid >> 3);
+            atomicMax(&hi, sid >> 3);
+            atomicAdd(&cnt, 1);
+        }
+    }
+    __syncthreads();
+    if (t == 0) {
+        const int nqt = (n_q[p] + 127) / 128;
+        int first = lo - slack < 0 ? 0 : lo - slack, end = hi + slack + 1 < nqt ? hi + slack + 1 : nqt;
+        if (cnt < DC_MIN_SURE || (long long)(end - first) * DC_BAND_CAP_DEN > (long long)nqt * DC_BAND_CAP_NUM) { first = 0; end = nqt; }
+        band[(p * T8 + panel) * 2] = first;
+        band[(p * T8 + panel) * 2 + 1] = end - first;
+        atomicAdd(&stats[p * 4 + 3], end - first);
+        if (panel == 0) stats[p * 4 + 0] = (na + stride - 1) / stride < MX6_SAMPLED_PANEL ? (na + stride - 1) / stride : MX6_SAMPLED_PANEL;
+    }
+}
+
+__global__ __launch_bounds__(256) void match_dc_settle_rows_kernel(int cap_a, int T8, int stride, int S, const int32_t *__restrict__ n_a,
+                                                                    const int32_t *__restrict__ n_q, const float *__restrict__ ws_m1,
+                                                                    const int32_t *__restrict__ ws_i1, const float *__restrict__ ws_m2,
+                                                                    const float *__restrict__ a_err, const float *__restrict__ q_err, float cut0,
+                                                                    const int32_t *__restrict__ band, float *__restrict__ r_m1,
+                                                                    int32_t *__restrict__ r_i1, float *__restrict__ r_m2, uint8_t *__restrict__ cls,
+                                                                    int32_t *__restrict__ n_open, int32_t *__restrict__ open_idx,
+                                                                    int32_t *__restrict__ stats)
+{
+    __shared__ int wave_cnt[4], wave_settled[4];
+    const int p = blockIdx.x, t = threadIdx.x, lane = t & 63, wave = t >> 6;
+    const int na = n_a[p], nqt = (n_q[p] + 127) / 128;
+    const float line = dc_sure_line(a_err, q_err, p, cut0);
+    const int R = (cap_a + 255) / 256;
+    uint8_t *cl = cls + (size_t)p * cap_a;
+    int mine = 0, settled = 0;
+    for (int i = 0; i < R; ++i) {
+        const int a = t * R + i;
+        if (a >= na || a >= cap_a) break;
+        const size_t arow = (size_t)p * cap_a + a;
+        if (a % stride == 0 && a / stride < MX6_SAMPLED_PANEL) { cl[a] = DC_COMPLETE; continue; }
+        const int32_t *b = band + (p * T8 + (a >> 10)) * 2;
+        const bool all = b[0] == 0 && b[1] == nqt;
+        float m1, m2;
+        int sid;
+        dc_merge(ws_m1, ws_i1, ws_m2, p, S, cap_a, a, m1, sid, m2);
+        uint8_t c;
+        if (all) c = DC_COMPLETE;
+        else if (m1 > line) { c = DC_SETTLED; m2 = INFINITY; ++settled; }
+        else { c = DC_OPEN; ++mine; }
+        cl[a] = c;
+        if (c != DC_OPEN) { r_m1[arow] = m1; r_i1[arow] = sid; r_m2[arow] = m2; }
+    }
+    int incl = mine, sett = settled;
+#pragma unroll
+    for (int off = 1; off < 64; off <<= 1) {
+        const int v = __shfl_up(incl, off);
+        if (lane >= off) incl += v;
+        sett += __shfl_xor(sett, off);
+    }
+    if (lane == 63) { wave_cnt[wave] = incl; wave_settled[wave] = sett; }
+    __syncthreads();
+    int off0 = incl - mine;
+    for (int w = 0; w < wave; ++w) off0 += wave_cnt[w];
+    for (int i = 0; i < R; ++i) {
+        const int a = t * R + i;
+        if (a >= na || a >= cap_a) break;
+        if (cl[a] == DC_OPEN) open_idx[(size_t)p * cap_a + off0++] = a;
+    }
+    if (t == 255) {
+        n_open[p] = off0;
+        stats[p * 4 + 1] = wave_settled[0] + wave_settled[1] + wave_settled[2] + wave_settled[3];
+        stats[p * 4 + 2] = off0;
+    }
+}
+
+__global__ __launch_bounds__(256) void match_dc_scatter_open_kernel(int cap_a, int S, const int32_t *__restrict__ n_open,
+                                                                     const int32_t *__restrict__ open_idx, const float *__restrict__ ws_m1,
+                                                                     const int32_t *__restrict__ ws_i1, const float *__restrict__ ws_m2,
+                                                                     float *__restrict__ r_m1, int32_t *__restrict__ r_i1, float *__restrict__ r_m2)
+{
+    const int p = blockIdx.y, sl = blockIdx.x * 256 + threadIdx.x;
+    if (sl >= n_open[p] || sl >= cap_a) return;
+    float m1, m2;
+    int sid;
+    dc_merge(ws_m1, ws_i1, ws_m2, p, S, cap_a, sl, m1, sid, m2);
+    const size_t arow = (size_t)p * cap_a + open_idx[(size_t)p * cap_a + sl];
+    r_m1[arow] = m1;
+    r_i1[arow] = sid;
+    r_m2[arow] = m2;
 }
 
 typedef float f32x32r __attribute__((ext_vector_type(32)));
@@ -491,6 +645,12 @@
     float *cs_max, *cs_m2;
     int32_t *cs_i1;
     int32_t *n_ambv0, *cs_gate;
+    bool dc_ok;
+    uint8_t *dc_rows;
+    float *dc_m1, *dc_m2, *dc_ws_m1, *dc_ws_m2;
+    int32_t *dc_i1, *dc_ws_i1, *dc_probe_idx, *dc_open_idx, *dc_band, *dc_n_probe, *dc_n_open, *dc_stats;
+    uint8_t *dc_cls;
+    size_t dc_zero_bytes;
     size_t lazy_zero_off, lazy_zero_bytes;
 };
 
@@ -498,6 +658,49 @@
 {
     const int cap_s0 = (corr_rows + 127) / 128 * 128;
     return cap_s0 < cap_a ? cap_s0 : cap_a;
+}
+
+bool dc_shape(int C, int cap_a, int corr_rows) { return C == 256 && corr_rows <= MX6_SAMPLED_PANEL && mx6_panels_per_pair(cap_a) >= 3; }
+int dc_probe_stride(int cap_a)
+{
+    static const int want = dev_env_int("ORYON_DC_STRIDE", 10);
+    const int s = (cap_a + MX6_SAMPLED_PANEL - 1) / MX6_SAMPLED_PANEL;
+    return s > want ? s : want;
+}
+int dc_band_splits(int B, int cap_a)
+{
+    static const int force = dev_env_int("ORYON_DC_BAND_SPLITS", 0);
+    const int u = B * mx6_panels_per_pair(cap_a), s = force > 0 ? force : (1280 + u - 1) / u;
+    return s < 1 ? 1 : s > 16 ? 16 : s;
+}
+int dc_open_splits(int B)
+{
+    static const int force = dev_env_int("ORYON_DC_OPEN_SPLITS", 0);
+    const int s = force > 0 ? force : (1024 + B - 1) / B;
+    return s < 1 ? 1 : s > 16 ? 16 : s;
+}
+size_t carve_dc(void *base, LazyWs &w, int B, int C, int cap_a)
+{
+    Carver carve(base);
+    const size_t rows = (size_t)B * cap_a, pairs = (size_t)B;
+    const size_t S = 16;
+    carve(w.dc_rows, rows * C);
+    carve(w.dc_m1, rows);
+    carve(w.dc_m2, rows);
+    carve(w.dc_i1, rows);
+    carve(w.dc_cls, rows);
+    carve(w.dc_open_idx, rows);
+    carve(w.dc_probe_idx, pairs * MX6_SAMPLED_PANEL);
+    carve(w.dc_band, pairs * mx6_panels_per_pair(cap_a) * 2);
+    carve(w.dc_ws_m1, rows * S);
+    carve(w.dc_ws_m2, rows * S);
+    carve(w.dc_ws_i1, rows * S);
+    const size_t zero_off = carve.off;
+    carve(w.dc_n_probe, pairs);
+    carve(w.dc_n_open, pairs);
+    carve(w.dc_stats, pairs * 4);
+    w.dc_zero_bytes = carve.off - zero_off;
+    return carve.off;
 }
 
 size_t carve_lazy(void *base, LazyWs &w, int B, int C, int cap_a, int cap_q, int S, int corr_rows)
@@ -534,6 +737,15 @@
     carve(w.cs_i1, triples);
     carve(w.n_ambv0, pairs);
     carve(w.cs_gate, pairs * mx6_panels_per_pair(cap_a));
+    w.dc_ok = false;
+    w.dc_stats = nullptr;
+    if (dc_shape(C, cap_a, corr_rows)) {
+        LazyWs sized;
+        if (carve_dc(nullptr, sized, B, C, cap_a) <= (size_t)B * cap_q * C * sizeof(__half)) {
+            carve_dc(w.q16, w, B, C, cap_a);
+            w.dc_ok = true;
+        }
+    }
     w.lazy_zero_off = carve.off;
     carve(w.pair_eager, pairs);
     carve(w.n_unc, pairs);
@@ -554,6 +766,13 @@
     return carve_lazy(nullptr, w, B, C, cap_a, cap_q, pick_split16(B, cap_a / MT16), corr_rows);
 }
 
+int32_t *oryon::match_dc_stats(void *workspace, int B, int C, int cap_a, int cap_q, int corr_rows)
+{
+    LazyWs w;
+    carve_lazy(workspace, w, B, C, cap_a, cap_q, pick_split16(B, cap_a / MT16), corr_rows);
+    return w.dc_ok ? w.dc_stats : nullptr;
+}
+
 namespace {
 constexpr const char *IMPL = "match_corrs_lazy_impl";
 
@@ -587,7 +806,7 @@
                            st, araw, m.C_true, m.HW, m.round_f16, m.C, m.cap_a, cap_c, count, idx, idx_stride, w.a_hat_c);
 }
 
-int lazy_route(const MatchCorrsArgs &m, const LazyWs &w, hipStream_t st, int use_x3, bool cascade)
+int lazy_route(const MatchCorrsArgs &m, const LazyWs &w, hipStream_t st, int use_x3, bool cascade, bool dc)
 {
     const int B = m.B, C = m.C, cap_a = m.cap_a, cap_q = m.cap_q, corr_rows = m.corr_rows;
     const bool nhwc = m.layout == ORYON_LAYOUT_NHWC;
@@ -617,12 +836,12 @@
     if (cascade) {
         const int csS = mx6_sampled_splits(B);
         hipLaunchKernelGGL(match_compact_rows_kernel, dim3(MX6_SAMPLED_PANEL / 16, B), dim3(256), 0, st, reinterpret_cast<const uint8_t *>(m.a_i8),
-                           C, cap_a, MX6_SAMPLED_PANEL, w.n_ambv, w.ambv_idx, corr_rows, w.cs_panel);
+                           C, cap_a, MX6_SAMPLED_PANEL, w.n_ambv, w.ambv_idx, corr_rows, w.cs_panel, MX6_SAMPLED_PANEL);
         launch_screen_mx6_sampled(st, w.cs_panel, reinterpret_cast<const uint8_t *>(m.q_i8), B, cap_q, w.n_ambv, m.n_q, csS, w.cs_max, w.cs_i1,
                                   w.cs_m2, m.C_true);
         hipLaunchKernelGGL(match_decide_sampled_kernel, dim3((MX6_SAMPLED_PANEL + 255) / 256, B), dim3(256), 0, st, cap_a, MX6_SAMPLED_PANEL, csS,
                            w.n_ambv, w.ambv_idx, corr_rows, w.cs_max, w.cs_i1, w.cs_m2, m.a_scale, m.q_eps_max, w.m_final, w.sid_final,
-                           w.margin, w.state, w.mark, w.n_ambv0);
+                           w.margin, w.state, w.mark, w.n_ambv0, dc ? m.min_dist : nullptr);
         hipLaunchKernelGGL(match_list_sampled_amb_kernel, dim3(B), dim3(256), 0, st, cap_a, w.state, w.pair_eager, m.n_sel, w.sel_rows,
                            corr_rows, w.mark, w.n_ambv, w.ambv_idx);
         if ((rc = check_launch(IMPL))) return rc;
@@ -696,11 +915,16 @@
     ORYON_CHECK_HIP(hipMemsetAsync(static_cast<char *>(m.workspace) + w.zero_off, 0, w.zero_bytes, st));
     if (m.force_eager) ORYON_CHECK_HIP(hipMemsetAsync(w.need_f32, 0, (size_t)B * sizeof(int32_t), st));
     ORYON_CHECK_HIP(hipMemsetAsync(static_cast<char *>(m.workspace) + w.lazy_zero_off, 0, w.lazy_zero_bytes, st));
+    if (w.dc_ok && m.fmt == 1) ORYON_CHECK_HIP(hipMemsetAsync(w.dc_n_probe, 0, w.dc_zero_bytes, st));
     const float cut0 = 1.0f - 2.0f * m.threshold;
     static const bool x3_env = dev_env_int("ORYON_AMB_X3", 1) != 0;
     const int use_x3 = (x3_env && C == 256 && !m.force_eager) ? 1 : 0;
     static const bool cascade_env = dev_env_int("ORYON_CASCADE", 1) != 0;
     const bool cascade = cascade_env && m.fmt == 1 && use_x3 && m.q_hi_lo != nullptr && w.cs_panel != nullptr;
+    const bool dc = m.cascade != 0 && m.fmt == 1 && use_x3 && m.q_hi_lo == nullptr && w.cs_panel != nullptr && w.dc_ok;
+    int S_dec = S;
+    const float *dec_m1 = w.ws_max, *dec_m2 = w.ws_m2;
+    const int32_t *dec_i1 = w.ws_i1;
     if (m.fmt == 1) {
         const uint8_t *a6 = reinterpret_cast<const uint8_t *>(m.a_i8), *q6 = reinterpret_cast<const uint8_t *>(m.q_i8);
         const int groups = ((B * S + 7) / 8) * 8 * T;
@@ -711,6 +935,33 @@
             hipLaunchKernelGGL(match_panel_settle_kernel, dim3(T8, B), dim3(256), 0, st, cap_a, T8, S, m.n_a, w.ws_max, w.ws_m2, m.a_scale,
                                m.q_eps_max, cut0, w.cs_gate);
             launch_screen_mx6(C, groups, T, st, a6, q6, B, cap_a, cap_q, m.n_a, m.n_q, S, w.ws_max, w.ws_i1, w.ws_m2, m.C_true, 1, w.cs_gate, 0);
+        } else if (dc) {
+            const int T8 = mx6_panels_per_pair(cap_a), stride = dc_probe_stride(cap_a), csS = mx6_sampled_splits(B);
+            const int Sb = dc_band_splits(B, cap_a), So = dc_open_splits(B);
+            static const int slack = dev_env_int("ORYON_DC_SLACK", DC_SLACK);
+            static const int open_panel = dev_env_int("ORYON_DC_OPEN_PANEL", 0) == 1024 ? 1024 : MX6_SAMPLED_PANEL;
+            hipLaunchKernelGGL(match_dc_probe_list_kernel, dim3(B), dim3(256), 0, st, stride, m.n_a, w.dc_n_probe, w.dc_probe_idx);
+            hipLaunchKernelGGL(match_compact_rows_kernel, dim3(MX6_SAMPLED_PANEL / 16, B), dim3(256), 0, st, a6, C, cap_a, MX6_SAMPLED_PANEL,
+                               w.dc_n_probe, w.dc_probe_idx, MX6_SAMPLED_PANEL, w.cs_panel, MX6_SAMPLED_PANEL);
+            launch_screen_mx6_sampled(st, w.cs_panel, q6, B, cap_q, w.dc_n_probe, m.n_q, csS, w.cs_max, w.cs_i1, w.cs_m2, m.C_true);
+            hipLaunchKernelGGL(match_dc_probe_band_kernel, dim3(T8, B), dim3(256), 0, st, cap_a, T8, stride, csS, m.n_a, m.n_q, w.cs_max, w.cs_i1,
+                               w.cs_m2, m.a_scale, m.q_eps_max, cut0, w.dc_m1, w.dc_i1, w.dc_m2, w.dc_band, w.dc_stats, slack);
+            launch_screen_mx6(C, ((B * Sb + 7) / 8) * 8 * T, T, st, a6, q6, B, cap_a, cap_q, m.n_a, m.n_q, Sb, w.dc_ws_m1, w.dc_ws_i1, w.dc_ws_m2, m.C_true,
+                              1, nullptr, 0, w.dc_band);
+            hipLaunchKernelGGL(match_dc_settle_rows_kernel, dim3(B), dim3(256), 0, st, cap_a, T8, stride, Sb, m.n_a, m.n_q, w.dc_ws_m1, w.dc_ws_i1,
+                               w.dc_ws_m2, m.a_scale, m.q_eps_max, cut0, w.dc_band, w.dc_m1, w.dc_i1, w.dc_m2, w.dc_cls, w.dc_n_open, w.dc_open_idx,
+                               w.dc_stats);
+            hipLaunchKernelGGL(match_compact_rows_kernel, dim3(cap_a / 16, B), dim3(256), 0, st, a6, C, cap_a, cap_a, w.dc_n_open, w.dc_open_idx,
+                               cap_a, w.dc_rows, open_panel);
+            if (open_panel == 1024)
+                launch_screen_mx6(C, ((B * So + 7) / 8) * 8 * T, T, st, w.dc_rows, q6, B, cap_a, cap_q, w.dc_n_open, m.n_q, So, w.dc_ws_m1, w.dc_ws_i1,
+                                  w.dc_ws_m2, m.C_true);
+            else
+                launch_screen_mx6_rows512(st, w.dc_rows, q6, B, cap_a, cap_q, w.dc_n_open, m.n_q, So, w.dc_ws_m1, w.dc_ws_i1, w.dc_ws_m2, m.C_true);
+            hipLaunchKernelGGL(match_dc_scatter_open_kernel, dim3(cap_a / 256, B), dim3(256), 0, st, cap_a, So, w.dc_n_open, w.dc_open_idx,
+                               w.dc_ws_m1, w.dc_ws_i1, w.dc_ws_m2, w.dc_m1, w.dc_i1, w.dc_m2);
+            S_dec = 1;
+            dec_m1 = w.dc_m1; dec_i1 = w.dc_i1; dec_m2 = w.dc_m2;
         } else {
             launch_screen_mx6(C, groups, T, st, a6, q6, B, cap_a, cap_q, m.n_a, m.n_q, S, w.ws_max, w.ws_i1, w.ws_m2, m.C_true);
         }
@@ -719,13 +970,13 @@
         screen8_step(m, S, m.n_a, w);
     }
     ORYON_CHECK_LAUNCH();
-    hipLaunchKernelGGL(match_decide_lite_kernel, dim3(cap_a / 256, B), dim3(256), 0, st, cap_a, m.n_a, S, w.ws_max, w.ws_i1, w.ws_m2, m.a_scale,
+    hipLaunchKernelGGL(match_decide_lite_kernel, dim3(cap_a / 256, B), dim3(256), 0, st, cap_a, m.n_a, S_dec, dec_m1, dec_i1, dec_m2, m.a_scale,
                        m.q_eps_max, cut0, sqrtf((float)m.C_true), (float)m.C_true, m.force_eager, m.fmt, use_x3, w.m_final, w.sid_final, w.margin,
                        w.state, m.valid, m.min_dist, m.argmin, w.pair_eager, w.n_unc, w.unc_idx, w.n_ambu, w.ambu_idx, w.need_f32_lazy,
                        w.n_amb_total);
     hipLaunchKernelGGL(match_mask_counts_kernel, dim3((B + 255) / 256), dim3(256), 0, st, B, m.n_a, w.pair_eager, w.n_a_eager, w.n_a_lazy);
     ORYON_CHECK_LAUNCH();
-    if (!m.force_eager) return lazy_route(m, w, st, use_x3, cascade);
+    if (!m.force_eager) return lazy_route(m, w, st, use_x3, cascade || dc, dc);
     const int rc = eager_route(m, w, S);
     if (rc) return rc;
     if (m.n_undecided) ORYON_CHECK_HIP(hipMemcpyAsync(m.n_undecided, w.n_amb, (size_t)B * sizeof(int32_t), hipMemcpyDeviceToDevice, st));
diff --git a/oryon_amd/csrc/screen_mx6.hip b/oryon_amd/csrc/screen_mx6.hip
--- a/oryon_amd/csrc/screen_mx6.hip
+++ b/oryon_amd/csrc/screen_mx6.hip
@@ -381,7 +381,8 @@
 __global__ __launch_bounds__(64 * WAVES, CP == 512 ? 1 : 2) void match_mx6_screen_w4_win_kernel(
     const uint8_t *__restrict__ a6, const uint8_t *__restrict__ q6, int B, int cap_a, int cap_q, const int32_t *__restrict__ n_a,
     const int32_t *__restrict__ n_q, int T, int S, float *__restrict__ ws_max, int32_t *__restrict__ ws_i1, float *__restrict__ ws_m2,
-    const int32_t *__restrict__ gate , int win )
+    const int32_t *__restrict__ gate , int win ,
+    const int32_t *__restrict__ band )
 {
     static_assert(CP == 256 || (CP == 512 && WAVES == 4), "geometries: C_pad 256 with 4 / 8 waves, C_pad 512 with 4 waves");
     constexpr int RB = CP, NAB = 4;
@@ -418,6 +419,12 @@
         qt_begin += k0;
         qt_end = qt_begin + win;
     }
+    if (band) {
+        const int first = band[(p * T + panel) * 2], cnt = band[(p * T + panel) * 2 + 1];
+        const int per = (cnt + S - 1) / S;
+        qt_begin = first + split * per;
+        qt_end = (qt_begin + per < first + cnt) ? qt_begin + per : first + cnt;
+    }
     const int t = threadIdx.x, lane = t & 63, wave = t >> 6, l31 = lane & 31, hi = lane >> 5;
     const char *qp = reinterpret_cast<const char *>(q6) + (size_t)p * cap_q * RB;
 
@@ -605,7 +612,7 @@
 template <int CP>
 void launch_screen_mx6_t(int groups, int T, hipStream_t st, const uint8_t *a6, const uint8_t *q6, int B, int cap_a, int cap_q, const int32_t *n_a,
                        const int32_t *n_q, int S, float *ws_max, int32_t *ws_i1, float *ws_m2, int kl = 0, bool gate_or_win = false,
-                       const int32_t *gate = nullptr, int win = 0)
+                       const int32_t *gate = nullptr, int win = 0, const int32_t *band = nullptr)
 {
     constexpr size_t dyn = 2 * screen8_tile_bytes(CP) > 65536 ? 2 * screen8_tile_bytes(CP) : 0;
     constexpr int W_ = CP == 512 ? 4 : 8;
@@ -628,7 +635,7 @@
             if (gate_or_win) {
 #define ORYON_LAUNCH_WIN(KLV)                                                                                                         \
     hipLaunchKernelGGL((match_mx6_screen_w4_win_kernel<CP, 8, KLV>), dim3(g8), dim3(512), 0, st, a6, q6, B, cap_a, cap_q, n_a, n_q, T8, S,   \
-                       ws_max, ws_i1, ws_m2, gate, win)
+                       ws_max, ws_i1, ws_m2, gate, win, band)
                 if (kl == 1) ORYON_LAUNCH_WIN(1);
                 else if (kl == 2) ORYON_LAUNCH_WIN(2);
                 else ORYON_LAUNCH_WIN(4);
@@ -675,27 +682,34 @@
 
 void launch_screen_mx6(int C, int groups, int T, hipStream_t st, const uint8_t *a6, const uint8_t *q6, int B, int cap_a, int cap_q,
                        const int32_t *n_a, const int32_t *n_q, int S, float *ws_max, int32_t *ws_i1, float *ws_m2, int C_true,
-                       int cascade, const int32_t *gate, int win)
+                       int cascade, const int32_t *gate, int win, const int32_t *band)
 {
     const int kl = (C == 256 && C_true > 0 && C_true <= 64) ? 1 : (C == 256 && C_true > 0 && C_true <= 128) ? 2 : 0;
-    if (C == 256) launch_screen_mx6_t<256>(groups, T, st, a6, q6, B, cap_a, cap_q, n_a, n_q, S, ws_max, ws_i1, ws_m2, kl, cascade != 0, gate, win);
+    if (C == 256) launch_screen_mx6_t<256>(groups, T, st, a6, q6, B, cap_a, cap_q, n_a, n_q, S, ws_max, ws_i1, ws_m2, kl, cascade != 0, gate, win, band);
     else launch_screen_mx6_t<512>(groups, T, st, a6, q6, B, cap_a, cap_q, n_a, n_q, S, ws_max, ws_i1, ws_m2);
+}
+
+void launch_screen_mx6_rows512(hipStream_t st, const uint8_t *a6_rows, const uint8_t *q6, int B, int cap_rows, int cap_q, const int32_t *n_rows,
+                               const int32_t *n_q, int S, float *ws_max, int32_t *ws_i1, float *ws_m2, int C_true)
+{
+    const int T = (cap_rows + 511) / 512;
+    const int groups = ((B * S + 7) / 8) * 8 * T;
+    const int kl = (C_true > 0 && C_true <= 64) ? 1 : (C_true > 0 && C_true <= 128) ? 2 : 0;
+    if (kl == 1)
+        hipLaunchKernelGGL((match_mx6_screen_w4_kernel<256, 4, 1>), dim3(groups), dim3(256), 0, st, a6_rows, q6, B, cap_rows, cap_q, n_rows, n_q, T, S,
+                           ws_max, ws_i1, ws_m2, static_cast<long long *>(nullptr));
+    else if (kl == 2)
+        hipLaunchKernelGGL((match_mx6_screen_w4_kernel<256, 4, 2>), dim3(groups), dim3(256), 0, st, a6_rows, q6, B, cap_rows, cap_q, n_rows, n_q, T, S,
+                           ws_max, ws_i1, ws_m2, static_cast<long long *>(nullptr));
+    else
+        hipLaunchKernelGGL((match_mx6_screen_w4_kernel<256, 4>), dim3(groups), dim3(256), 0, st, a6_rows, q6, B, cap_rows, cap_q, n_rows, n_q, T, S,
+                           ws_max, ws_i1, ws_m2, static_cast<long long *>(nullptr));
 }
 
 void launch_screen_mx6_sampled(hipStream_t st, const uint8_t *a6_panel, const uint8_t *q6, int B, int cap_q, const int32_t *n_rows,
                                const int32_t *n_q, int S, float *ws_max, int32_t *ws_i1, float *ws_m2, int C_true)
 {
-    const int groups = ((B * S + 7) / 8) * 8;
-    const int kl = (C_true > 0 && C_true <= 64) ? 1 : (C_true > 0 && C_true <= 128) ? 2 : 0;
-    if (kl == 1)
-        hipLaunchKernelGGL((match_mx6_screen_w4_kernel<256, 4, 1>), dim3(groups), dim3(256), 0, st, a6_panel, q6, B, 512, cap_q, n_rows, n_q, 1, S,
-                           ws_max, ws_i1, ws_m2, static_cast<long long *>(nullptr));
-    else if (kl == 2)
-        hipLaunchKernelGGL((match_mx6_screen_w4_kernel<256, 4, 2>), dim3(groups), dim3(256), 0, st, a6_panel, q6, B, 512, cap_q, n_rows, n_q, 1, S,
-                           ws_max, ws_i1, ws_m2, static_cast<long long *>(nullptr));
-    else
-        hipLaunchKernelGGL((match_mx6_screen_w4_kernel<256, 4>), dim3(groups), dim3(256), 0, st, a6_panel, q6, B, 512, cap_q, n_rows, n_q, 1, S,
-                           ws_max, ws_i1, ws_m2, static_cast<long long *>(nullptr));
-}
-
-}
+    launch_screen_mx6_rows512(st, a6_panel, q6, B, MX6_SAMPLED_PANEL, cap_q, n_rows, n_q, S, ws_max, ws_i1, ws_m2, C_true);
+}
+
+}
diff --git a/oryon_amd/engine.py b/oryon_amd/engine.py
--- a/oryon_amd/engine.py
+++ b/oryon_amd/engine.py
@@ -71,7 +71,7 @@
 
     def __init__(self, solver: Optional[PointDSC], cfg: "MatchPoseConfig", key: Tuple, dev: torch.device, overlap: int, n_slots: int = 6,
                  gather_sets: int = 2, reg_streams: int = 2, reg_lag: int = 0, screen: int = 1, x3_prefetch: int = 1,
-                 stream_roles: int = 0):
+                 stream_roles: int = 0, screen_cascade: int = 1):
         B, C, FH, FW, HA, WA, HQ, WQ, layout = key
         self.key, self.dev = key, dev
         if overlap >= 2:
@@ -89,7 +89,7 @@
                                       reg_lag=reg_lag if overlap else 0, screen=screen,
                                       sample_first=int(cfg.sample_first) if cfg.sample_first and cfg.sample_first > 0 else 0,
                                       x3_prefetch=int(bool(x3_prefetch)) if (C <= 256 and screen == 1) else 0,
-                                      stream_roles=int(stream_roles), solver=int(ransac), ransac_max_iter=int(cfg.ransac_max_iter),
+                                      stream_roles=int(stream_roles), screen_cascade=int(bool(screen_cascade)), solver=int(ransac), ransac_max_iter=int(cfg.ransac_max_iter),
                                       ransac_match_err=float(cfg.ransac_match_err), ransac_fix_percent=float(cfg.ransac_fix_percent))
         self.cfg_sig = _cfg_sig(cfg, overlap)
         need = lib().oryon_engine_arena_bytes(ctypes.byref(self.ecfg), handle)
@@ -161,6 +161,11 @@
         check(lib().oryon_engine_x3_steps(self._h, ctypes.byref(n)))
         return n.value
 
+    def cascade_stats(self) -> Tensor:
+        out = torch.zeros((self.geo["B"], 4), dtype=torch.int32)
+        check(lib().oryon_engine_cascade_stats(self._h, out.data_ptr()), "oryon_engine_cascade_stats")
+        return out
+
     def feedback(self) -> Optional[Tuple[int, int, int]]:
         st, und, na = ctypes.c_int64(), ctypes.c_int64(), ctypes.c_int64()
         check(lib().oryon_engine_feedback(self._h, ctypes.byref(st), ctypes.byref(und), ctypes.byref(na)))
@@ -202,7 +207,7 @@
         self.result_views = result_views
         self._native: Optional[NativeStep] = None
         self._inflight: Dict[int, Dict[str, Tensor]] = {}
-        self.native_geometry = dict(n_slots=6, gather_sets=2, reg_streams=2, reg_lag=0, screen=1, x3_prefetch=1, stream_roles=0)
+        self.native_geometry = dict(n_slots=6, gather_sets=2, reg_streams=2, reg_lag=0, screen=1, x3_prefetch=1, stream_roles=0, screen_cascade=1)
         self.native_timing = False
         self._reg_stream = None
         self.reg_streams = 2
```

Result: faster. 22340 (median of 6 runs) (+12.2%).
